# neuromodulation/py_neuromodulation

Hardware: AMD Instinct MI355X
Metric: windows/sec (all features), 256 ch @ 1 kHz (higher is better)
Workload: dtype f32; 1 GPU; 256ch/GPU @1kHz, W=1000, hop=100, 1024 hops/step, all 9 hot-path features, 4 bands, notch50+CAR, z-score normalisation; channels_per_gpu=256, features_per_window=9984, parallelism=channel-shard x1, no collective

## Files before the change

### py_neuromodulation_amd/csrc/nmx_api.hip

```cpp
#include <chrono>
#include <map>
#include <unordered_map>
#include <thread>
#include <hip/hip_runtime.h>

#include "nmx_k_bank.h"
#include "nmx_k_bank_w64.h"
#include "nmx_k_bank_w64d.h"
#include "nmx_k_bank_w64e.h"
#include "nmx_k_bursts.h"
#include "nmx_k_burst_fill.h"
#include "nmx_k_kalman.h"
#include "nmx_k_norm.h"
#include "nmx_k_power.h"
#include "nmx_k_prep.h"
#include "nmx_k_rawnorm.h"
#include "nmx_k_resample.h"
#include "nmx_k_resample64.h"
#include "nmx_k_sharpwave.h"
#include "nmx_k_specmm.h"
#include "nmx_k_timeosc.h"
#include "nmx_k_timeosc_w510.h"

#include <cstdlib>
#include <map>
#include <mutex>
#include <string>

extern __shared__ __attribute__((aligned(16))) float nmx_smem[];

__global__ void __launch_bounds__(256) nmx_kern_timeosc(const NmxTimeOscArgs A) {
  const int item = blockIdx.x;
  nmx_time_osc_item(A, item / A.n_channels, item % A.n_channels, nmx_smem);
}
__global__ void __launch_bounds__(256) nmx_kern_bank(const NmxBankArgs A, int n_items) {
  for (int item = blockIdx.x; item < n_items; item += gridDim.x)
    nmx_bank_item(A, item / A.n_channels, item % A.n_channels, nmx_smem, (int)blockIdx.x);
}
template <int CH>
__global__ void __launch_bounds__(256) nmx_kern_burst_thr(const NmxBurstThrArgs A) {
  __builtin_amdgcn_s_setprio(3);
  const int item = blockIdx.x;
  nmx_burst_thr_item<CH>(A, item / A.n_bands, item % A.n_bands, nmx_smem);
}
__global__ void __launch_bounds__(NMX_FILL_NT) nmx_kern_burst_fill(const NmxBurstThrArgs A, int n2, unsigned short* slots) {
  const int item = blockIdx.x;
  nmx_burst_fill_item(A, item / A.n_bands, item % A.n_bands, n2, slots, nmx_smem);
}
__global__ void __launch_bounds__(NMX_FILL_NT) nmx_kern_burst_fill_sort(const NmxBurstThrArgs A, int n2, unsigned short* slots, float* sorted) {
  const int item = blockIdx.x;
  nmx_burst_fill_sort_item(A, item / A.n_bands, item % A.n_bands, n2, slots, sorted, nmx_smem);
}
__global__ void __launch_bounds__(64) nmx_kern_burst_fill_walk(const NmxBurstThrArgs A, int n2, const unsigned short* slots, const float* sorted) {
  const int item = blockIdx.x;
  nmx_burst_fill_walk_item(A, item / A.n_bands, item % A.n_bands, n2, slots, sorted, nmx_smem);
}
__global__ void __launch_bounds__(1024) nmx_kern_burst_thr_wide(const NmxBurstThrArgs A) {
  const int item = blockIdx.x;
  nmx_burst_thr_item<64>(A, item / A.n_bands, item % A.n_bands, nmx_smem);
}
__global__ void __launch_bounds__(NMX_THR_TILE_NT) nmx_kern_burst_thr_tiled(const NmxBurstThrArgs A) {
  const int item = blockIdx.x;
  nmx_burst_thr_walk<1, true>(A, item / A.n_bands, item % A.n_bands, nmx_smem);
}
extern "C" void nmx_timeosc_fixed_launch128(const NmxTimeOscArgs* A, int n_items, size_t lds, hipStream_t s);
extern "C" void nmx_hilbert_fixed_launch128(const NmxHilbertArgs* A, long long n_items, size_t lds, hipStream_t s);
extern "C" void nmx_wave_launch_burst_stat(const NmxBurstStatArgs* A, NmxBurstStatKind kind, int n_items, size_t lds, hipStream_t s);
extern "C" void nmx_wave_launch_sharp(const NmxSharpArgs* A, int n_items, size_t lds, hipStream_t s);
__global__ void __launch_bounds__(256) nmx_kern_reref(const NmxRerefArgs A) {
  nmx_reref_tile(A, (long long)blockIdx.x * 256 + threadIdx.x, (int)blockIdx.y * NMX_REREF_ROWS);
}
__global__ void __launch_bounds__(256) nmx_kern_resample(const NmxResampleArgs A) {
  const int item = blockIdx.x;
  nmx_resample_item(A, item / A.n_channels, item % A.n_channels, nmx_smem);
}
__global__ void __launch_bounds__(64) nmx_kern_rawnorm_stats(const NmxRawNormArgs A) {
  nmx_rawnorm_stats_item(A, (int)blockIdx.x);
}
__global__ void __launch_bounds__(NMX_RAWNORM_ORDER_NT) nmx_kern_rawnorm_order(const NmxRawNormArgs A) {
  extern __shared__ __attribute__((aligned(16))) float nmx_smem_rn[];
  nmx_rawnorm_order_item(A, (int)blockIdx.x, nmx_smem_rn);
}
__global__ void __launch_bounds__(256) nmx_kern_rawnorm_apply(const NmxRawNormArgs A) {
  nmx_rawnorm_apply(A, (long long)blockIdx.x * 256 + threadIdx.x);
}
__global__ void __launch_bounds__(64) nmx_kern_kalman(const NmxKalmanArgs A) {
  const int i = (int)(blockIdx.x * 64 + threadIdx.x);
  nmx_kalman_item(A, i / A.n_bands, i % A.n_bands);
}
__global__ void __launch_bounds__(64) nmx_kern_norm(const NmxNormArgs A) {
  nmx_norm_column(A, (int)(blockIdx.x * 64 + threadIdx.x));
}
__global__ void __launch_bounds__(64) nmx_kern_norm_seg_hist(const NmxNormArgs A, const NmxNormScan S) {
  nmx_norm_seg_hist(A, S, (int)blockIdx.y, (int)(blockIdx.x * 64 + threadIdx.x));
}
__global__ void __launch_bounds__(64) nmx_kern_norm_seg_batch(const NmxNormArgs A, const NmxNormScan S) {
  nmx_norm_seg_batch(A, S, (int)blockIdx.y, (int)(blockIdx.x * 64 + threadIdx.x));
}
__global__ void __launch_bounds__(64) nmx_kern_norm_seg_offsets(const NmxNormArgs A, const NmxNormScan S) {
  nmx_norm_seg_offsets(A, S, (int)(blockIdx.x * 64 + threadIdx.x));
}
__global__ void __launch_bounds__(256) nmx_kern_norm_cell(const NmxNormArgs A, const NmxNormScan S) {
  nmx_norm_scan_cell(A, S, (int)blockIdx.x, (int)(blockIdx.y * 256 + threadIdx.x));
}
__global__ void __launch_bounds__(256) nmx_kern_norm_ring(const NmxNormArgs A, const NmxNormScan S) {
  nmx_norm_scan_ring(A, S, (int)blockIdx.x, (int)(blockIdx.y * 256 + threadIdx.x));
}
__global__ void __launch_bounds__(256) nmx_kern_power_prep(const NmxPowerPrepArgs P) {
  nmx_power_prep_at(P, (int)blockIdx.x, (int)(blockIdx.y * 256 + threadIdx.x));
}
__global__ void __launch_bounds__(64) nmx_kern_power(const NmxPowerArgs A) {
  nmx_power_cell(A, (int)blockIdx.x, (int)(blockIdx.y * 64 + threadIdx.x));
}
__global__ void __launch_bounds__(256) nmx_kern_power_ring(const NmxPowerPrepArgs P) {
  nmx_power_ring_at(P, (int)blockIdx.x, (int)(blockIdx.y * 256 + threadIdx.x));
}
template <int NW>
__global__ void __launch_bounds__(64 * NW) nmx_kern_car(const NmxCarArgs A) {
  __shared__ double red[64 * NW];
  nmx_car_tile<NW>(A, (long long)blockIdx.x * 64, red);
}
__global__ void __launch_bounds__(256) nmx_kern_reref_struct(const NmxRerefStructArgs A) {
  __shared__ double red[NMX_RS_GROUPS * 256];
  nmx_reref_struct_tile(A, (long long)blockIdx.x * 64, red);
}
__global__ void __launch_bounds__(256) nmx_kern_shift(const NmxShiftArgs A) {
  nmx_shift_sample(A, (long long)blockIdx.x * 256 + threadIdx.x, (int)blockIdx.y);
}
__global__ void __launch_bounds__(64) nmx_kern_nanmask(const NmxNanMaskArgs A) {
  const int item = blockIdx.x;
  nmx_nanmask_item(A, item / A.C_in, item % A.C_in, nmx_smem);
}
__global__ void __launch_bounds__(256) nmx_kern_tap(const NmxTapArgs A) {
  const int item = blockIdx.x;
  nmx_tap_item(A, item / A.C, item % A.C);
}

static thread_local int g_stage = 0;
static thread_local std::string g_stage_kernels[16];
extern "C" void nmxi_note_kernel(const char* name) {
  std::string& s = g_stage_kernels[g_stage & 15];
  if (s.find(name) != std::string::npos) return;
  if (!s.empty()) s += " + ";
  s += name;
}
static void be_stage(int st) { g_stage = st; }
static void be_stage_reset() { for (auto& s : g_stage_kernels) s.clear(); }
static std::string be_stage_kernels(int st) { return g_stage_kernels[st & 15]; }

typedef hipStream_t be_stream_t;
struct be_timer_t {
  hipEvent_t a = nullptr, b = nullptr;
  bool used = false;
};

static thread_local std::string g_be_err;
static thread_local int g_be_rc = 0;
static int nmx_fail(int code, const std::string& msg);
static int be_hip(hipError_t e, const char* what) {
  if (e == hipSuccess) return 0;
  return nmx_fail(NMX_E_HIP, std::string(what) + ": " + hipGetErrorString(e));
}
#define BE_TRY(call) do { hipError_t e_ = (call); if (e_ != hipSuccess && !g_be_rc) g_be_rc = be_hip(e_, #call); } while (0)

static int be_device_count() {
  int n = 0;
  if (hipGetDeviceCount(&n) != hipSuccess) return 0;
  return n;
}
static int be_set_device(int dev) { return be_hip(hipSetDevice(dev), "hipSetDevice"); }
static int be_cu_count(int dev) {
  int n = 0;
  return hipDeviceGetAttribute(&n, hipDeviceAttributeMultiprocessorCount, dev) == hipSuccess && n > 0 ? n : 256;
}
struct NmxDevIdle { void* p; long long gen; };
struct NmxDevPool {
  std::mutex m;
  std::multimap<std::pair<int, size_t>, NmxDevIdle> idle;
  std::map<void*, std::pair<int, size_t>> live;
  size_t cached = 0, cap = 0;
  long long gen = 0;
  bool cap_read = false;
};
static NmxDevPool& be_dev_pool() { static NmxDevPool* p = new NmxDevPool(); return *p; }
static void be_dev_pool_flush(NmxDevPool& D, size_t keep = 0, long long older_than = -1) {
  for (auto it = D.idle.begin(); it != D.idle.end();) {
    const bool old = older_than >= 0 && it->second.gen <= older_than;
    if (!(old || (older_than < 0 && D.cached > keep))) { ++it; continue; }
    (void)hipFree(it->second.p);
    D.cached -= it->first.second;
    it = D.idle.erase(it);
  }
}
static void be_dev_pool_cap(NmxDevPool& D) {
  if (D.cap_read) return;
  const char* v = getenv("NMX_DEVICE_POOL_MB");
  D.cap = (size_t)((v && v[0] >= '0' && v[0] <= '9') ? atoll(v) : 8192) << 20;
  D.cap_read = true;
}
static void* be_alloc(size_t n) {
  NmxDevPool& D = be_dev_pool();
  int dev = 0;
  if (hipGetDevice(&dev) != hipSuccess) dev = 0;
  const size_t want = ((n ? n : 4) + 255) & ~(size_t)255;
  std::lock_guard<std::mutex> lk(D.m);
  be_dev_pool_cap(D);
  auto it = D.idle.find(std::make_pair(dev, want));
  if (it != D.idle.end()) {
    void* p = it->second.p;
    D.idle.erase(it);
    D.cached -= want;
    D.live[p] = std::make_pair(dev, want);
    return p;
  }
  void* p = nullptr;
  if (hipMalloc(&p, want) != hipSuccess) {
    (void)hipGetLastError();
    be_dev_pool_flush(D);
    if (hipMalloc(&p, want) != hipSuccess) { (void)hipGetLastError(); return nullptr; }
  }
  D.live[p] = std::make_pair(dev, want);
  return p;
}
static void be_free(void* p) {
  if (!p) return;
  NmxDevPool& D = be_dev_pool();
  (void)hipDeviceSynchronize();
  std::lock_guard<std::mutex> lk(D.m);
  auto it = D.live.find(p);
  if (it == D.live.end()) { (void)hipFree(p); return; }
  const std::pair<int, size_t> key = it->second;
  D.live.erase(it);
  size_t cap = D.cap;
  if (cap && key.second >= (size_t)(64u << 20)) {
    size_t fr = 0, tot = 0;
    if (hipMemGetInfo(&fr, &tot) == hipSuccess) cap = std::min(cap, (fr + D.cached) / 8);
    else (void)hipGetLastError();
  }
  if (cap && D.cached + key.second <= cap) {
    D.idle.emplace(key, NmxDevIdle{p, D.gen});
    D.cached += key.second;
    return;
  }
  (void)hipFree(p);
}
static void be_dev_pool_age() {
  NmxDevPool& D = be_dev_pool();
  static const long long keep_plans = [] {
    const char* v = getenv("NMX_POOL_KEEP_PLANS");
    return (long long)((v && v[0] >= '0' && v[0] <= '9') ? atoll(v) : 4);
  }();
  std::lock_guard<std::mutex> lk(D.m);
  D.gen += 1;
  if (D.gen > keep_plans) be_dev_pool_flush(D, 0, D.gen - keep_plans - 1);
}
static long long be_dev_pool_trim(long long keep_bytes) {
  NmxDevPool& D = be_dev_pool();
  std::lock_guard<std::mutex> lk(D.m);
  const size_t before = D.cached;
  be_dev_pool_flush(D, keep_bytes > 0 ? (size_t)keep_bytes : 0);
  return (long long)(before - D.cached);
}
static void* be_host_alloc(size_t n) {
  void* p = nullptr;
  if (hipHostMalloc(&p, n, hipHostMallocPortable)    != hipSuccess) return nullptr;
  return p;
}
static void be_host_free(void* p) { (void)hipHostFree(p); }
static void be_h2d_sync(void* d, const void* s, size_t n) { BE_TRY(hipMemcpy(d, s, n, hipMemcpyHostToDevice)); }
static void be_d2h_sync(void* d, const void* s, size_t n) { BE_TRY(hipMemcpy(d, s, n, hipMemcpyDeviceToHost)); }
static void be_memset_sync(void* d, int v, size_t n) { BE_TRY(hipMemset(d, v, n)); }
static void be_h2d_async(void* d, const void* s, size_t n, be_stream_t st) {
  BE_TRY(hipMemcpyAsync(d, s, n, hipMemcpyHostToDevice, st));
}
static void be_d2h_async(void* d, const void* s, size_t n, be_stream_t st) {
  BE_TRY(hipMemcpyAsync(d, s, n, hipMemcpyDeviceToHost, st));
}
static void be_h2d_2d_async(void* d, size_t dpitch, const void* s, size_t spitch, size_t width,
                            size_t height, be_stream_t st) {
  BE_TRY(hipMemcpy2DAsync(d, dpitch, s, spitch, width, height, hipMemcpyHostToDevice, st));
}
static void be_d2h_2d_async(void* d, size_t dpitch, const void* s, size_t spitch, size_t width,
                            size_t height, be_stream_t st) {
  BE_TRY(hipMemcpy2DAsync(d, dpitch, s, spitch, width, height, hipMemcpyDeviceToHost, st));
}
static void be_memset_async(void* d, int v, size_t n, be_stream_t st) { BE_TRY(hipMemsetAsync(d, v, n, st)); }
static void be_host_fn(be_stream_t st, void (*fn)(void*), void* arg) { BE_TRY(hipLaunchHostFunc(st, fn, arg)); }
static int be_sync(be_stream_t st) { return be_hip(hipStreamSynchronize(st), "hipStreamSynchronize"); }
static int be_sync_watch(be_stream_t st, const std::string* kernels, int n_lists) {
  static const double limit = [] {
    const char* v = getenv("NMX_SYNC_TIMEOUT_S");
    return (v && ((v[0] >= '0' && v[0] <= '9') || v[0] == '.')) ? atof(v) : 300.0;
  }();
  const auto t0 = std::chrono::steady_clock::now();
  for (;;) {
    const hipError_t q = hipStreamQuery(st);
    if (q == hipSuccess) return 0;
    if (q != hipErrorNotReady) return be_hip(q, "hipStreamQuery");
    (void)hipGetLastError();
    const double el = std::chrono::duration<double>(std::chrono::steady_clock::now() - t0).count();
    if (limit > 0.0 && el > limit) {
      std::string msg = "the device did not finish a batch within " + std::to_string((int)limit) + " s (NMX_SYNC_TIMEOUT_S); kernels of the last launch sequence:";
      for (int i = 1; i < n_lists; ++i)
        if (kernels && !kernels[i].empty()) msg += " [stage " + std::to_string(i) + ": " + kernels[i] + "]";
      return nmx_fail(NMX_E_HIP, msg);
    }
    if (el > 1e-3) std::this_thread::sleep_for(std::chrono::microseconds(50));
  }
}
static void be_sync_quiet(be_stream_t st) { if (hipStreamSynchronize(st) != hipSuccess) (void)hipGetLastError(); }
struct NmxStreamPool {
  std::mutex mu;
  std::vector<hipStream_t> idle[2];
  std::unordered_map<hipStream_t, int> cls;
};
static NmxStreamPool& be_stream_pool(int dev) {
  static std::mutex mu;
  static std::map<int, NmxStreamPool*> pools;
  std::lock_guard<std::mutex> lk(mu);
  NmxStreamPool*& p = pools[dev];
  if (!p) p = new NmxStreamPool();
  return *p;
}
static int be_stream_pool_cap() {
  static int cap = -1;
  if (cap < 0) { const char* v = getenv("NMX_STREAM_POOL"); cap = v ? std::max(0, atoi(v)) : 32; }
  return cap;
}
static be_stream_t be_stream_make(int klass) {
  int dev = 0;
  (void)hipGetDevice(&dev);
  NmxStreamPool& P = be_stream_pool(dev);
  hipStream_t s = nullptr;
  {
    std::lock_guard<std::mutex> lk(P.mu);
    if (!P.idle[klass].empty()) { s = P.idle[klass].back(); P.idle[klass].pop_back(); P.cls[s] = klass; return s; }
  }
  if (klass == 1) {
    int lo = 0, hi = 0;
    if (!(hipDeviceGetStreamPriorityRange(&lo, &hi) == hipSuccess &&
          hipStreamCreateWithPriority(&s, hipStreamNonBlocking, hi) == hipSuccess)) {
      s = nullptr;
      (void)hipGetLastError();
    }
  }
  if (!s) BE_TRY(hipStreamCreateWithFlags(&s, hipStreamNonBlocking));
  if (s) { std::lock_guard<std::mutex> lk(P.mu); P.cls[s] = klass; }
  return s;
}
static be_stream_t be_stream_create() { return be_stream_make(0); }
static void be_stream_destroy(be_stream_t s) {
  if (!s) return;
  int dev = 0;
  (void)hipGetDevice(&dev);
  NmxStreamPool& P = be_stream_pool(dev);
  {
    std::lock_guard<std::mutex> lk(P.mu);
    auto it = P.cls.find(s);
    if (it != P.cls.end()) {
      const int klass = it->second;
      P.cls.erase(it);
      if ((int)P.idle[klass].size() < be_stream_pool_cap() && hipStreamQuery(s) == hipSuccess) { P.idle[klass].push_back(s); return; }
      (void)hipGetLastError();
    }
  }
  (void)hipStreamDestroy(s);
}
static be_stream_t be_stream_create_high() { return be_stream_make(1); }
typedef hipEvent_t be_event_t;
static void be_event_create(be_event_t& e) { BE_TRY(hipEventCreateWithFlags(&e, hipEventDisableTiming)); }
static void be_event_destroy(be_event_t& e) { if (e) (void)hipEventDestroy(e); }
static void be_event_record(be_event_t& e, be_stream_t s) { BE_TRY(hipEventRecord(e, s)); }
static void be_stream_wait(be_stream_t s, be_event_t& e) { BE_TRY(hipStreamWaitEvent(s, e, 0)); }
static void be_timer_create(be_timer_t& t) {
  BE_TRY(hipEventCreate(&t.a));
  BE_TRY(hipEventCreate(&t.b));
}
static void be_timer_destroy(be_timer_t& t) {
  if (t.a) (void)hipEventDestroy(t.a);
  if (t.b) (void)hipEventDestroy(t.b);
}
static void be_timer_start(be_timer_t& t, be_stream_t s) { BE_TRY(hipEventRecord(t.a, s)); t.used = false; }
static void be_timer_stop(be_timer_t& t, be_stream_t s) { BE_TRY(hipEventRecord(t.b, s)); t.used = true; }
static float be_timer_elapsed(be_timer_t& t) {
  if (!t.used) return 0.f;
  float ms = 0.f;
  if (hipEventSynchronize(t.b) != hipSuccess) return -1.f;
  if (hipEventElapsedTime(&ms, t.a, t.b) != hipSuccess) return -1.f;
  return ms;
}
static int be_check_launch() {
  hipError_t e = hipGetLastError();
  if (e != hipSuccess) return be_hip(e, "kernel launch");
  int rc = g_be_rc;
  g_be_rc = 0;
  return rc;
}

template <typename K>
static void be_allow_lds(K kern) {
  (void)hipFuncSetAttribute((const void*)kern, hipFuncAttributeMaxDynamicSharedMemorySize, 160 * 1024);
}
static void be_init_once() {
  static unsigned long long seen = 0;
  if (!nmx_first_on_device(seen)) return;
  be_allow_lds(nmx_kern_timeosc);
  be_allow_lds(nmx_kern_bank);
  be_allow_lds(nmx_kern_resample);
  be_allow_lds(nmx_kern_burst_thr<32>);
  be_allow_lds(nmx_kern_burst_thr<64>);
  be_allow_lds(nmx_kern_burst_thr<128>);
  be_allow_lds(nmx_kern_burst_thr_wide);
  be_allow_lds(nmx_kern_burst_thr_tiled);
  be_allow_lds(nmx_kern_burst_fill);
  be_allow_lds(nmx_kern_burst_fill_sort);
  be_allow_lds(nmx_kern_rawnorm_order);
}

extern "C" void nmx_wave_launch_scan(const NmxTimeOscArgs* A, int n_items, hipStream_t s);
extern "C" void nmx_wave_launch_timeosc_w1000_low(const NmxTimeOscArgs* A, int n_items, int n_cu, hipStream_t s);
extern "C" void nmx_wave_launch_timeosc_w1000(const NmxTimeOscArgs* A, int n_items, hipStream_t s);
extern "C" void nmx_wave_launch_timeosc_w510(const NmxTimeOscArgs* A, int n_items, hipStream_t s);
extern "C" void nmx_wave_launch_timeosc_stft500(const NmxTimeOscArgs* A, int n_items, hipStream_t s);
extern "C" void nmx_specmm_launch(const NmxTimeOscArgs* A, int n_items, int n_cu, hipStream_t s);
extern "C" void nmx_wave_launch_timeosc_w1000_todo(const NmxTimeOscArgs* A, int n_items, hipStream_t s);
extern "C" void nmx_timeosc_long_launch(const NmxTimeOscArgs* A, int n_items, hipStream_t s);
static void be_launch_timeosc(const NmxTimeOscArgs& A, NmxTimeOscKind kind, int n_items, int nt, size_t lds, int n_cu, be_stream_t s) {
  be_init_once();
  switch (kind) {
    case NMX_TO_SCAN: nmx_wave_launch_scan(&A, n_items, s); return;
    case NMX_TO_SPECMM: nmx_specmm_launch(&A, n_items, n_cu, s); return;
    case NMX_TO_W1000_LOW: nmx_wave_launch_timeosc_w1000_low(&A, n_items, n_cu, s); return;
    case NMX_TO_W1000: nmx_wave_launch_timeosc_w1000(&A, n_items, s); return;
    case NMX_TO_STFT500: nmx_wave_launch_timeosc_stft500(&A, n_items, s); return;
    case NMX_TO_W510: nmx_wave_launch_timeosc_w510(&A, n_items, s); return;
    case NMX_TO_FIXED128: nmx_timeosc_fixed_launch128(&A, n_items, lds, s); return;
    case NMX_TO_LONG: nmx_timeosc_long_launch(&A, n_items, s); return;
    case NMX_TO_GENERIC:
      hipLaunchKernelGGL(nmx_kern_timeosc, dim3(n_items), dim3(nt), lds, s, A);
      nmxi_note_kernel("nmx_kern_timeosc");
      return;
  }
}
static void be_launch_timeosc_redo(const NmxTimeOscArgs& A, int n_items, be_stream_t s) {
  nmx_wave_launch_timeosc_w1000_todo(&A, n_items, s);
}
static void be_launch_bank(const NmxBankArgs& A, int n_items, int nt, size_t lds, be_stream_t s) {
  be_init_once();
  const int grid = (A.partitioned && n_items > NMX_UPS_SLOTS) ? NMX_UPS_SLOTS : n_items;
  hipLaunchKernelGGL(nmx_kern_bank, dim3(grid), dim3(nt), lds, s, A, n_items);
  nmxi_note_kernel("nmx_kern_bank");
}
extern "C" void nmx_w64_launch_rd64(const NmxBankW64Args*, int, size_t, int, hipStream_t);
extern "C" void nmx_w64x2_launch_rd64(const NmxBankW64Args*, int, int, hipStream_t);
extern "C" void nmx_w64c_launch_rd64(const NmxBankW64Args*, int, int, hipStream_t);
extern "C" void nmx_w64d_launch_rd64(const NmxBankW64Args*, int, int, hipStream_t);
extern "C" void nmx_w64e_launch_rd64(const NmxBankW64Args*, int, int, hipStream_t);
extern "C" void nmx_wave_launch_sharp_todo(const NmxSharpArgs* A, int n_items, size_t lds, const unsigned char* todo,
                                           hipStream_t s);
static void be_launch_bank_w64(const NmxBankW64Args& A, int n_items, size_t lds, int n_cu, be_stream_t s) {
  switch ((NmxFirKernel)A.kernel) {
    case NMX_FIR_X2: nmx_w64x2_launch_rd64(&A, n_items, n_cu, s); return;
    case NMX_FIR_PAIR_C: nmx_w64c_launch_rd64(&A, n_items, n_cu, s); return;
    case NMX_FIR_PAIR_D: nmx_w64d_launch_rd64(&A, n_items, n_cu, s); return;
    case NMX_FIR_PAIR_E: nmx_w64e_launch_rd64(&A, n_items, n_cu, s); return;
    case NMX_FIR_ONE: nmx_w64_launch_rd64(&A, n_items, lds, n_cu, s); return;
  }
}
extern "C" void nmx_w64e_launch_fused_rd64(const NmxBankW64Args*, const NmxBankW64Args*, int, int, int, hipStream_t);
static void be_launch_notch_bank_fused(const NmxBankW64Args& F, const NmxBankW64Args& N, bool g_lds, int n_items, int n_cu,
                                       be_stream_t s) {
  nmx_w64e_launch_fused_rd64(&F, &N, g_lds ? 1 : 0, n_items, n_cu, s);
}
extern "C" void nmx_wave_launch_sharp_dense(const NmxSharpArgs* A, NmxSharpKind kind, int n_items, hipStream_t s);
extern "C" void nmx_wave_launch_sharp_slab(const NmxSharpArgs* A, int n_items, const unsigned char* todo, hipStream_t s);
static void be_launch_sharp(const NmxSharpArgs& A, NmxSharpKind kind, int n_items, size_t lds, be_stream_t s) {
  be_init_once();
  switch (kind) {
    case NMX_SHARP_LIST: nmx_wave_launch_sharp(&A, n_items, lds, s); return;
    case NMX_SHARP_SLAB: nmx_wave_launch_sharp_slab(&A, n_items, nullptr, s); return;
    case NMX_SHARP_DENSE_LIST: nmx_wave_launch_sharp_dense(&A, kind, n_items, s); nmx_wave_launch_sharp_todo(&A, n_items, lds, A.todo, s); return;
    case NMX_SHARP_DENSE_SLAB: nmx_wave_launch_sharp_dense(&A, kind, n_items, s); nmx_wave_launch_sharp_slab(&A, n_items, A.todo, s); return;
  }
}
extern "C" void nmx_wave_launch_hilbert_w500(const NmxHilbertArgs* A, long long n_items, hipStream_t s);
extern "C" void nmx_wave_launch_hilbert_w1000(const NmxHilbertArgs* A, long long n_items, hipStream_t s);
extern "C" void nmx_hilbert_long_launch(const NmxHilbertArgs* A, long long n_items, hipStream_t s);
static void be_launch_hilbert(const NmxHilbertArgs& A, NmxHilbertKind kind, long long n_items, size_t lds, be_stream_t s) {
  be_init_once();
  if (kind == NMX_HIL_W500) nmx_wave_launch_hilbert_w500(&A, n_items, s);
  else if (kind == NMX_HIL_W1000) nmx_wave_launch_hilbert_w1000(&A, n_items, s);
  else if (kind == NMX_HIL_LONG) nmx_hilbert_long_launch(&A, n_items, s);
  else nmx_hilbert_fixed_launch128(&A, n_items, lds, s);
}
extern "C" void nmx_wave_launch_burst_thr(const NmxBurstThrArgs* A, int n_items, int nr, bool list_lds, size_t lds, hipStream_t s);
static void be_launch_burst_thr(const NmxBurstThrArgs& A, const NmxBurstWalk& K, const NmxBurstWalkSeg& g, int n_items, int nt, size_t lds,
                                be_stream_t s) {
  be_init_once();
  if (g.kind == NMX_WALK_WAVE) { nmx_wave_launch_burst_thr(&A, n_items, K.nr, g.list_lds, g.list_lds ? K.lds_list : K.lds, s); return; }
  const int chunk = (A.K + nt - 1) / nt;
  if (nmx_burst_thr_tiled(A.K)) { hipLaunchKernelGGL(nmx_kern_burst_thr_tiled, dim3(n_items), dim3(NMX_THR_TILE_NT), lds, s, A); nmxi_note_kernel("nmx_kern_burst_thr_tiled"); }
  else if (nt > 256) { hipLaunchKernelGGL(nmx_kern_burst_thr_wide, dim3(n_items), dim3(1024), lds, s, A); nmxi_note_kernel("nmx_kern_burst_thr_wide"); }
  else if (chunk <= 32) { hipLaunchKernelGGL(nmx_kern_burst_thr<32>, dim3(n_items), dim3(nt), lds, s, A); nmxi_note_kernel("nmx_kern_burst_thr<32>"); }
  else if (chunk <= 64) { hipLaunchKernelGGL(nmx_kern_burst_thr<64>, dim3(n_items), dim3(nt), lds, s, A); nmxi_note_kernel("nmx_kern_burst_thr<64>"); }
  else { hipLaunchKernelGGL(nmx_kern_burst_thr<128>, dim3(n_items), dim3(nt), lds, s, A); nmxi_note_kernel("nmx_kern_burst_thr<128>"); }
}
static void be_launch_burst_fill(const NmxBurstThrArgs& A, int n_items, unsigned short* slots, float* sorted, bool split, be_stream_t s) {
  be_init_once();
  int n2 = 2048;
  while (n2 < A.W + (A.n_windows - 1) * A.overlap) n2 <<= 1;
  const size_t lds_walk = nmx_burst_fill_walk_lds(n2, A.n_windows);
  if (split && lds_walk <= 48 * 1024) {
    hipLaunchKernelGGL(nmx_kern_burst_fill_sort, dim3(n_items), dim3(NMX_FILL_NT), nmx_burst_fill_sort_lds(n2), s, A, n2, slots, sorted);
    hipLaunchKernelGGL(nmx_kern_burst_fill_walk, dim3(n_items), dim3(64), lds_walk, s, A, n2, (const unsigned short*)slots,
                       (const float*)sorted);
    nmxi_note_kernel("nmx_kern_burst_fill_sort");
    nmxi_note_kernel("nmx_kern_burst_fill_walk");
    return;
  }
  hipLaunchKernelGGL(nmx_kern_burst_fill, dim3(n_items), dim3(NMX_FILL_NT), nmx_burst_fill_lds(n2), s, A, n2, slots);
  nmxi_note_kernel("nmx_kern_burst_fill");
}
static void be_launch_burst_stat(const NmxBurstStatArgs& A, NmxBurstStatKind kind, int n_items, size_t lds, be_stream_t s) {
  be_init_once();
  nmx_wave_launch_burst_stat(&A, kind, n_items, lds, s);
}
static void be_launch_reref(const NmxRerefArgs& A, be_stream_t s) {
  dim3 grid((unsigned)((A.T + 255) / 256), (unsigned)((A.C + NMX_REREF_ROWS - 1) / NMX_REREF_ROWS));
  hipLaunchKernelGGL(nmx_kern_reref, grid, dim3(256), 0, s, A);
  nmxi_note_kernel("nmx_kern_reref");
}
static void be_launch_resample(const NmxResampleArgs& A, int n_items, int nt, size_t lds, be_stream_t s) {
  be_init_once();
  hipLaunchKernelGGL(nmx_kern_resample, dim3(n_items), dim3(nt), lds, s, A);
  nmxi_note_kernel("nmx_kern_resample");
}
static void be_launch_rawnorm(const NmxRawNormArgs& A, be_stream_t s) {
  be_init_once();
  if (A.method >= NMX_RAWNORM_MEDIAN && A.method != NMX_RAWNORM_POWER) {
    const size_t lds = A.lists ? (size_t)8 * NMX_RAWNORM_ORDER_NT + 4 * (2 * NMX_RAWNORM_ORDER_NT + 272)
                               : (size_t)24 * A.max_list + 8 * NMX_RAWNORM_ORDER_NT;
    hipLaunchKernelGGL(nmx_kern_rawnorm_order, dim3(A.n_channels), dim3(NMX_RAWNORM_ORDER_NT), lds, s, A);
    const long long n = (long long)A.n_windows * A.n_channels * A.W;
    hipLaunchKernelGGL(nmx_kern_rawnorm_apply, dim3((unsigned)((n + 255) / 256)), dim3(256), 0, s, A);
    nmxi_note_kernel("nmx_kern_rawnorm_order + nmx_kern_rawnorm_apply");
    return;
  }
  hipLaunchKernelGGL(nmx_kern_rawnorm_stats, dim3(A.n_channels), dim3(64), 0, s, A);
  const long long n = (long long)A.n_windows * A.n_channels * A.W;
  hipLaunchKernelGGL(nmx_kern_rawnorm_apply, dim3((unsigned)((n + 255) / 256)), dim3(256), 0, s, A);
  nmxi_note_kernel("nmx_kern_rawnorm_stats + nmx_kern_rawnorm_apply");
}
static void be_launch_kalman(const NmxKalmanArgs& A, be_stream_t s) {
  const int n = A.n_channels * A.n_bands;
  hipLaunchKernelGGL(nmx_kern_kalman, dim3((unsigned)((n + 63) / 64)), dim3(64), 0, s, A);
  nmxi_note_kernel("nmx_kern_kalman");
}
static void be_launch_norm(const NmxNormArgs& A, be_stream_t s) {
  hipLaunchKernelGGL(nmx_kern_norm, dim3((unsigned)((A.n_cols + 63) / 64)), dim3(64), 0, s, A);
}
static void be_launch_norm_scan(const NmxNormArgs& A, const NmxNormScan& S, be_stream_t s) {
  const unsigned cb = (unsigned)((A.n_cols + 63) / 64);
  const dim3 cells((unsigned)A.n_rows, (unsigned)((A.n_cols + 255) / 256));
  if (S.n_hseg) hipLaunchKernelGGL(nmx_kern_norm_seg_hist, dim3(cb, (unsigned)S.n_hseg), dim3(64), 0, s, A, S);
  hipLaunchKernelGGL(nmx_kern_norm_seg_batch, dim3(cb, (unsigned)S.n_bseg), dim3(64), 0, s, A, S);
  hipLaunchKernelGGL(nmx_kern_norm_seg_offsets, dim3(cb), dim3(64), 0, s, A, S);
  hipLaunchKernelGGL(nmx_kern_norm_cell, cells, dim3(256), 0, s, A, S);
  hipLaunchKernelGGL(nmx_kern_norm_ring, cells, dim3(256), 0, s, A, S);
}
static void be_launch_power(const NmxPowerPrepArgs& P, const NmxPowerArgs& A, be_stream_t s) {
  const unsigned gy = (unsigned)((P.n_cols + 255) / 256);
  hipLaunchKernelGGL(nmx_kern_power_prep, dim3((unsigned)(P.have + P.n_rows), gy), dim3(256), 0, s, P);
  hipLaunchKernelGGL(nmx_kern_power, dim3((unsigned)A.n_rows, (unsigned)((A.n_cols + 63) / 64)), dim3(64), 0, s, A);
  hipLaunchKernelGGL(nmx_kern_power_ring, dim3((unsigned)P.n_rows, gy), dim3(256), 0, s, P);
}
static void be_launch_car(const NmxCarArgs& A, be_stream_t s) {
  if (A.T <= 4096 && A.C >= 64) hipLaunchKernelGGL(nmx_kern_car<16>, dim3((unsigned)((A.T + 63) / 64)), dim3(1024), 0, s, A);
  else hipLaunchKernelGGL(nmx_kern_car<4>, dim3((unsigned)((A.T + 63) / 64)), dim3(256), 0, s, A);
  nmxi_note_kernel("nmx_kern_car");
}
static void be_launch_reref_struct(const NmxRerefStructArgs& A, be_stream_t s) {
  hipLaunchKernelGGL(nmx_kern_reref_struct, dim3((unsigned)((A.T + 63) / 64)), dim3(256), 0, s, A);
  nmxi_note_kernel("nmx_kern_reref_struct");
}
static void be_launch_shift(const NmxShiftArgs& A, be_stream_t s) {
  hipLaunchKernelGGL(nmx_kern_shift, dim3((unsigned)((A.T + 255) / 256), (unsigned)A.C), dim3(256), 0, s, A);
  nmxi_note_kernel("nmx_kern_shift");
}
__global__ void __launch_bounds__(256) nmx_kern_reref64(const NmxReref64Args A) {
  nmx_reref64_tile(A, (long long)blockIdx.x * 256 + threadIdx.x, (int)blockIdx.y * NMX_REREF64_ROWS);
}
static void be_launch_reref64(const NmxReref64Args& A, be_stream_t s) {
  hipLaunchKernelGGL(nmx_kern_reref64, dim3((unsigned)((A.T + 255) / 256), (unsigned)((A.C + NMX_REREF64_ROWS - 1) / NMX_REREF64_ROWS)),
                     dim3(256), 0, s, A);
}
__global__ void __launch_bounds__(256) nmx_kern_rs64_elem(const NmxResample64Args A, int mode, const NmxCplx64* src, NmxCplx64* dst) {
  nmx_rs64_elem(A, mode, src, dst, (int)blockIdx.y, (long long)blockIdx.x * 256 + threadIdx.x);
}
__global__ void __launch_bounds__(256) nmx_kern_rs64_pass(const NmxCplx64* src, NmxCplx64* dst, long long ld, long long n, long long ns,
                                                          long long st, int sign) {
  nmx_rs64_pass(src, dst, ld, n, ns, st, sign, (int)blockIdx.y, (long long)blockIdx.x * 256 + threadIdx.x);
}
static void be_launch_rs64_elem(const NmxResample64Args& A, int mode, const NmxCplx64* src, NmxCplx64* dst, long long n, int rows,
                                be_stream_t s) {
  hipLaunchKernelGGL(nmx_kern_rs64_elem, dim3((unsigned)((n + 255) / 256), (unsigned)rows), dim3(256), 0, s, A, mode, src, dst);
}
static void be_launch_rs64_pass(const NmxCplx64* src, NmxCplx64* dst, long long ld, long long n, long long ns, long long st, int sign,
                                int rows, be_stream_t s) {
  hipLaunchKernelGGL(nmx_kern_rs64_pass, dim3((unsigned)((n / 2 + 255) / 256), (unsigned)rows), dim3(256), 0, s, src, dst, ld, n, ns,
                     st, sign);
}
static void be_launch_nanmask(const NmxNanMaskArgs& A, int n_items, be_stream_t s) {
  hipLaunchKernelGGL(nmx_kern_nanmask, dim3(n_items), dim3(64), 64 * sizeof(float), s, A);
}
static void be_launch_tap(const NmxTapArgs& A, int n_items, be_stream_t s) {
  hipLaunchKernelGGL(nmx_kern_tap, dim3(n_items), dim3(256), 0, s, A);
}

#include "nmx_engine.inc"
```

### py_neuromodulation_amd/csrc/nmx_common.h

```cpp
#pragma once

#include <math.h>
#include <stdint.h>

#ifdef NMX_HOST_EMU
struct float2 {
  float x, y;
};
static inline float2 make_float2(float x, float y) { return float2{x, y}; }
#define NMX_DEV static inline
#define NMX_DEVM inline
#define NMX_TID 0
#define NMX_NT 1
#define NMX_SYNC() ((void)0)
#define NMX_GLOBAL_FENCE() ((void)0)
#define NMX_RESTRICT
#else
#include <hip/hip_runtime.h>
#define NMX_DEV __device__ __forceinline__
#define NMX_DEVM __device__ __forceinline__
#ifdef NMX_NT_FIXED
#define NMX_TID ((int)(threadIdx.x & 63))
#define NMX_NT 64
#elif defined(NMX_BLOCK_FIXED)
#define NMX_TID ((int)threadIdx.x)
#define NMX_NT NMX_BLOCK_FIXED
#else
#define NMX_TID ((int)threadIdx.x)
#define NMX_NT ((int)blockDim.x)
#endif
#define NMX_WAVE_FENCE() asm volatile("s_waitcnt lgkmcnt(0)" ::: "memory")
#if defined(NMX_NT_FIXED) && defined(NMX_SYNC_GLOBAL)
#define NMX_SYNC()                                                       \
  do {                                                                   \
    __builtin_amdgcn_fence(__ATOMIC_ACQ_REL, "workgroup");               \
    asm volatile("s_waitcnt vmcnt(0) lgkmcnt(0)" ::: "memory");          \
  } while (0)
#elif defined(NMX_NT_FIXED)
#define NMX_SYNC() NMX_WAVE_FENCE()
#elif defined(NMX_BLOCK_FIXED)
#define NMX_SYNC()                                        \
  do {                                                    \
    if (NMX_BLOCK_FIXED <= 64) { NMX_WAVE_FENCE(); }      \
    else { __syncthreads(); }                             \
  } while (0)
#else
#define NMX_SYNC()                                   \
  do {                                               \
    if (blockDim.x <= 64) { NMX_WAVE_FENCE(); }      \
    else { __syncthreads(); }                        \
  } while (0)
#endif
#define NMX_RESTRICT __restrict__
#define NMX_GLOBAL_FENCE() __threadfence_block()
extern "C" void nmxi_note_kernel(const char* name);
static inline bool nmx_first_on_device(unsigned long long& seen) {
  int d = 0;
  if (hipGetDevice(&d) != hipSuccess || d < 0 || d > 63) return true;
  if ((seen >> d) & 1ull) return false;
  seen |= 1ull << d;
  return true;
}
#endif

#ifdef NMX_HOST_EMU
static inline int nmx_uniform_i(int v) { return v; }
static inline long long nmx_uniform_ll(long long v) { return v; }
#else
__device__ __forceinline__ int nmx_uniform_i(int v) { return __builtin_amdgcn_readfirstlane(v); }
__device__ __forceinline__ long long nmx_uniform_ll(long long v) {
  const unsigned lo = (unsigned)__builtin_amdgcn_readfirstlane((int)(unsigned)(v & 0xffffffffll));
  const unsigned hi = (unsigned)__builtin_amdgcn_readfirstlane((int)(unsigned)((unsigned long long)v >> 32));
  return (long long)(((unsigned long long)hi << 32) | lo);
}
#endif

#define NMX_MAX_STAGES 12
#define NMX_MAX_BANDS_DEV 16
#define NMX_SMM_NG 63
#define NMX_SMM_TAB_FLOATS (4 * NMX_SMM_NG * 64)
#define NMX_MAX_FILTERS_DEV 24
#define NMX_MAX_SW_COMBOS_DEV 48

struct NmxFftStage {
  int radix;
  int ns;
  int m;
  unsigned magic;
  int tw_step;
};

struct NmxFft {
  int n;
  int nstages;
  NmxFftStage st[NMX_MAX_STAGES];
  const float2* tw;
  const float2* twr;
};

struct NmxCols {
  int base, ch_stride, a_stride, b_stride;
};

struct NmxOsc {
  int enabled;
  int n;
  int nfreq;
  int k_lo, k_hi;
  int nseg;
  int step;
  int half;
  int complex_full;
  int log_transform;
  unsigned estimators;
  int n_est;
  int return_spectrum;
  float scale;
  float log10_scale;
  int bin_lo[NMX_MAX_BANDS_DEV], bin_hi[NMX_MAX_BANDS_DEV];
  float inv_bins[NMX_MAX_BANDS_DEV];
  NmxCols cols, psd_cols;
  NmxFft fft;
  const float* win;
  const float2* wdc;
  int nadd;
  int split_d, sub_m;
  const float2* tw_n;
};

struct NmxTimeOscArgs {
  int stft_per_wave;
  const float* x;
  long long ch_stride;
  long long win_stride;
  const long long* starts;
  float* out;
  int n_outputs;
  int n_channels;
  int W;
  int n_bands;
  int clean_on_load;
  unsigned features;
  NmxCols hjorth_cols, raw_cols, ll_cols;
  NmxOsc fft, welch, stft;
  int off_x, off_a, off_b, off_spec, off_red, lds_floats;
  const float* w500_tab;
  const unsigned short* w510_tab;
  const float* smm_tab;
  int smm_k0;
  int starts_mod4;
  const float* dcf;
  unsigned short* todo;
  int long_mode;
  int long_nb;
  int long_spec_slab;
  int slab_floats;
  int slab_blocks;
  float* slab;
};

enum NmxTimeOscKind { NMX_TO_SCAN, NMX_TO_SPECMM, NMX_TO_W1000_LOW, NMX_TO_W1000, NMX_TO_STFT500, NMX_TO_W510, NMX_TO_FIXED128, NMX_TO_GENERIC, NMX_TO_LONG };
enum NmxHilbertKind { NMX_HIL_W500, NMX_HIL_W1000, NMX_HIL_FIXED128, NMX_HIL_LONG };
enum NmxBurstStatKind { NMX_BSTAT_REG16, NMX_BSTAT_REG16_SPARSE, NMX_BSTAT_REG32, NMX_BSTAT_REG32_SPARSE, NMX_BSTAT_GENERIC, NMX_BSTAT_SCAN };
enum NmxSharpKind { NMX_SHARP_LIST, NMX_SHARP_DENSE_LIST, NMX_SHARP_SLAB, NMX_SHARP_DENSE_SLAB };
enum NmxFirKernel { NMX_FIR_ONE, NMX_FIR_X2, NMX_FIR_PAIR_C, NMX_FIR_PAIR_D, NMX_FIR_PAIR_E };

#define NMXD_F_HJORTH (1u << 0)
#define NMXD_F_RAW (1u << 1)
#define NMXD_F_BANDPOWER (1u << 2)
#define NMXD_F_STFT (1u << 3)
#define NMXD_F_FFT (1u << 4)
#define NMXD_F_WELCH (1u << 5)
#define NMXD_F_SHARPWAVE (1u << 6)
#define NMXD_F_BURSTS (1u << 7)
#define NMXD_F_LINELENGTH (1u << 8)

#define NMXD_EST_MEAN 1u
#define NMXD_EST_MEDIAN 2u
#define NMXD_EST_STD 4u
#define NMXD_EST_MAX 8u
```

### py_neuromodulation_amd/csrc/nmx_engine.inc

```

#include <algorithm>
#include <chrono>
#include <cmath>
#include <cstdio>
#include <cstdlib>
#include <cstring>
#include <map>
#include <string>
#include <thread>
#include <deque>
#include <functional>
#include <mutex>
#include <condition_variable>
#include <pthread.h>
#include <vector>

#include "../../include/nmx.h"
#include "nmx_k_coh.h"
#include "nmx_k_proj.h"

static thread_local std::string g_nmx_err;
static int nmx_fail(int code, const std::string& msg) {
  g_nmx_err = msg;
  return code;
}
#define NMX_REQUIRE(cond, msg) \
  do { if (!(cond)) return nmx_fail(NMX_E_INVALID, std::string(msg)); } while (0)

#ifdef NMX_HOST_EMU
static void be_launch_timeosc(const NmxTimeOscArgs& A, NmxTimeOscKind, int n, int nt, size_t lds, int, be_stream_t s) { be_launch_timeosc(A, n, nt, lds, s); }
static void be_launch_hilbert(const NmxHilbertArgs& A, NmxHilbertKind, long long n, size_t lds, be_stream_t s) { be_launch_hilbert(A, n, 128, lds, s); }
static void be_launch_bank_w64(const NmxBankW64Args& A, int n, size_t lds, int, be_stream_t s) { be_launch_bank_w64(A, n, lds, s); }
static void be_launch_burst_thr(const NmxBurstThrArgs& A, const NmxBurstWalk&, const NmxBurstWalkSeg&, int n, int nt, size_t lds, be_stream_t s) {
  be_launch_burst_thr(A, n, nt, lds, s);
}
static void be_launch_burst_fill(const NmxBurstThrArgs& A, int n, unsigned short* slots, float* sorted, bool, be_stream_t s) {
  be_launch_burst_fill(A, n, slots, sorted, s);
}
static void be_launch_burst_stat(const NmxBurstStatArgs& A, NmxBurstStatKind, int n, size_t lds, be_stream_t s) { be_launch_burst_stat(A, n, lds, s); }
static void be_launch_sharp(const NmxSharpArgs& A, NmxSharpKind, int n, size_t lds, be_stream_t s) { be_launch_sharp(A, n, lds, s); }
static int be_cu_count(int) { return 256; }
#endif

namespace {

constexpr double kPi = 3.14159265358979323846;

template <void* (*Alloc)(size_t), void (*Free)(void*)>
struct Block {
  void* p = nullptr;
  size_t cap = 0;
  Block() = default;
  Block(const Block&) = delete;
  Block& operator=(const Block&) = delete;
  ~Block() { if (p) Free(p); }
  bool regrow(size_t bytes) {
    if (p) Free(p);
    p = Alloc(bytes);
    cap = p ? bytes : 0;
    return p != nullptr;
  }
};
using Buf = Block<be_alloc, be_free>;
using HostBuf = Block<be_host_alloc, be_host_free>;

#include "nmx_engine_sched.inc"

enum Stage {
  ST_BATCH = 0,
  ST_PREP = 1,
  ST_TIMEOSC = 2,
  ST_BANK = 3,
  ST_BURSTS = 4,
  ST_SHARP = 5,
  ST_BANK2 = 6,
  ST_COH = 7,
  ST_PROJ = 8,
  ST_COUNT
};

struct WinView {
  const float* x;
  long long ch_stride, win_stride;
  const long long* starts;
  int clean;
};
template <class Args>
void view_into(Args& A, const WinView& v) {
  A.x = v.x; A.ch_stride = v.ch_stride; A.win_stride = v.win_stride; A.starts = v.starts; A.clean_on_load = v.clean;
}
void view_into(NmxTapArgs& A, const WinView& v) {
  A.x = v.x; A.ch_stride = v.ch_stride; A.win_stride = v.win_stride; A.starts = v.starts; A.clean = v.clean;
}
WinView dense_view(const void* y, int C, int w) { return WinView{(const float*)y, w, (long long)C * w, nullptr, 0}; }

struct FrontStage {
  float* d_R = nullptr;
  bool car = false;
  float car_diag = 0.f, car_off = 0.f;
  bool structured = false;
  NmxRerefStructArgs rst{};
  Buf x_ref;
};
struct TimeOscStage {
  NmxTimeOscArgs a{};
  NmxTimeOscKind kind = NMX_TO_GENERIC;
  bool takes_dc = true;
  int nt = 64;
  Buf todo;
};
struct CohStage {
  NmxCohArgs a{};
};
struct ResampleStage {
  NmxResampleArgs a{};
  int nt = 256;
  Buf y;
};

struct FirLaunch {
  unsigned mask = 0;
  Stage stage = ST_BANK;
  NmxFirKernel kernel = NMX_FIR_ONE;
  bool pipelined = false;
  const float* hc = nullptr;
  const float* twc = nullptr;
  bool fused = false;
};
struct FirStage {
  NmxBankArgs a{};
  bool w64 = false;
  NmxBankW64Args w{};
  std::vector<FirLaunch> launches;
  bool takes_dc = true;
};

struct BurstStage {
  NmxHilbertArgs hil{};
  NmxBurstThrArgs bthr{};
  NmxBurstStatArgs bstat{};
  NmxHilbertKind hil_kind = NMX_HIL_FIXED128;
  bool own_hilbert = false;
  bool sparse = false;
  bool sparse_count = false;
  long long env_tail_rows = 0, env_rows = 0;
  NmxBurstStatKind stat_kind = NMX_BSTAT_GENERIC;
  NmxBurstWalk walk{};
  bool fill_split = true;
  int nt_thr = 256;
  long long seen = 0;
  float* d_top = nullptr;
  long long* d_counts = nullptr;
  size_t top_bytes = 0, counts_bytes = 0;
  float* d_floor = nullptr;
  Buf env[2], thr[2];
  Buf env_full[2];
  Buf yb;
  Buf slots;
  int fill_hops(int nw) const { return walk.fill && seen == 0 ? nmx_burst_fill_hops(bthr, nw) : 0; }
};
struct SharpStage {
  NmxSharpArgs a{};
  NmxSharpKind kind = NMX_SHARP_LIST;
  Buf swy[2], todo[2];
  Buf slab;
};
struct KalmanStage {
  NmxKalmanArgs a{};
  double* d_state = nullptr;
  size_t bytes = 0;
};
struct RawNormStage {
  NmxRawNormArgs a{};
  long long hops = 0;
  bool sorted_valid = false;
  size_t ring_bytes = 0, cnt_bytes = 0, len_bytes = 0;
  Buf x_rn, mean, scale;
  Buf qt, qn;
};

struct Plan {
  nmx_plan_desc d;
  std::vector<std::vector<double>> taps;
  std::vector<double> notch_taps, ref_matrix;
  std::vector<double> notch_taps_used;
  int device = 0;
  int n_cu = 256;
  Schedule sched;
  int host_chunk_windows = 512;
  int host_first_chunk = 128;
  int norm_chunk_windows = 384;
  std::vector<void*> tables;
  ~Plan() { for (void* t : tables) be_free(t); }
  std::map<int, NmxFft> fft_cache;
  std::map<int, const float2*> twn_cache;
  FrontStage front;
  FirStage bank;
  bool have_bank = false;
  FirStage notch;
  bool have_notch = false;
  int notch_bank_fuse = 0;
  std::vector<FirStage> pre;
  const float* w64e_tw = nullptr;
  const float* w500_tab = nullptr;
  BurstStage bursts;
  bool have_bursts = false;
  SharpStage sharp;
  bool have_sharp = false;
  TimeOscStage timeosc;
  bool have_timeosc = false;
  CohStage coherence;
  bool have_coh = false;
  int nt_bank = 256;
  int chunk_windows = 1024;
  int burst_handoff_mb = 2048;
  bool tiny_inline = true;
  bool starts_mod4 = false;
  Buf tap;
  Buf x_in, x_in2[2], x_pf[2], y_notch, out, starts, mask;
  HostBuf win_pin;
  KalmanStage kalman;
  bool have_kalman = false;
  ResampleStage resample;
  bool have_resample = false;
  RawNormStage rawnorm;
  bool have_rawnorm = false;
  std::vector<std::vector<double>> pre_taps;
  int w_in = 0;
  be_timer_t timers[ST_COUNT];
  std::string kernels[ST_COUNT];
  nmx_norm* norm = nullptr;
  nmx_proj* proj = nullptr;
  bool dc_ok = false;
  bool dc_auto = true;
  bool dc_host_set = false, dc_learned = false, dc_dirty = false;
  bool dc_active = false;
  bool dc_sub_active = false;
  double dc_gain = 1.0;
  std::vector<double> dc_host;
  std::vector<float> dc_sub_h;
  std::vector<double> dc_pre_h;
  float* d_dc_sub = nullptr;
  float* d_dc_pref = nullptr;
  float* d_dc_nanv = nullptr;
  Buf x_dc;
  const volatile int64_t* pipe_in_ready = nullptr;
  volatile int64_t* pipe_out_done = nullptr;
  struct Progress { volatile int64_t* dst; int64_t value; };
  std::vector<Progress> pipe_marks;
};

static thread_local double g_ensure_scale = 1.0;
int ensure(Buf& b, size_t bytes) {
  if (bytes <= b.cap) return 0;
  if (g_ensure_scale > 1.0) bytes = (size_t)((double)bytes * g_ensure_scale) + 256;
  const size_t want = bytes + bytes / 8;
  if (!b.regrow(want)) return nmx_fail(NMX_E_NOMEM, "device allocation of " + std::to_string(want) + " bytes failed");
  return 0;
}

void* plan_alloc(Plan& P, size_t bytes) {
  void* d = be_alloc(bytes ? bytes : 4);
  if (d) P.tables.push_back(d);
  return d;
}
void* upload(Plan& P, const void* src, size_t bytes) {
  void* d = plan_alloc(P, bytes);
  if (d && bytes) be_h2d_sync(d, src, bytes);
  return d;
}

int env_int(const char* name, int dflt) {
  const char* v = getenv(name);
  return (v && v[0] >= '0' && v[0] <= '9') ? atoi(v) : dflt;
}

#include "nmx_engine_dc.inc"
#include "nmx_engine_plan_spectral.inc"
#include "nmx_engine_plan_bursts.inc"
#include "nmx_engine_plan_fir.inc"
#include "nmx_engine_plan_state.inc"

}

#include "nmx_engine_abi.inc"
#include "nmx_engine_run.inc"
#include "nmx_engine_norm.inc"
#include "nmx_engine_proj.inc"
#include "nmx_engine_host.inc"
```

### py_neuromodulation_amd/csrc/nmx_engine_run.inc

```
static int run_prep_stages(Plan& P, WinView& v, int nw, be_stream_t s, const NmxBankArgs* fuse_bank = nullptr) {
  const int C = P.d.n_channels, Wi = P.w_in;
  int rc;
  for (size_t i = 0; i < P.pre.size(); ++i) {
    Buf& dst = P.x_pf[i & 1];
    if ((rc = ensure(dst, (size_t)nw * C * Wi * sizeof(float)))) return rc;
    NmxBankArgs A = P.pre[i].a;
    view_into(A, v);
    A.out = nullptr; A.sw_out = (float*)dst.p;
    launch_fir_stage(P, P.pre[i], A, nw * C, s);
    v = dense_view(dst.p, C, Wi);
  }
  if (P.have_notch) {
    if ((rc = ensure(P.y_notch, (size_t)nw * C * Wi * sizeof(float)))) return rc;
    NmxBankArgs A = P.notch.a;
    view_into(A, v);
    A.out = nullptr; A.y_out = (float*)P.y_notch.p;
#ifndef NMX_HOST_EMU
    if (fuse_bank) launch_notch_bank_fused(P, A, *fuse_bank, nw * C, s);
    else
#endif
    launch_fir_stage(P, P.notch, A, nw * C, s);
    v = dense_view(P.y_notch.p, C, Wi);
  }
  if (P.have_resample && (rc = launch_resample(P, v, nw, s))) return rc;
  if (P.have_rawnorm && (rc = run_rawnorm(P, v, nw, s))) return rc;
  return 0;
}

static int run_chunk(Plan& P, const BatchSched& b, const float* d_x, long long ldx, long long lo, long long hi,
                     const long long* d_starts, int nw, float* d_out, bool timed, float* d_pre = nullptr,
                     const int64_t* h_starts = nullptr, be_event_t* samples_free = nullptr, bool* samples_freed = nullptr) {
  const nmx_plan_desc& d = P.d;
  const int C = d.n_channels, W = d.window;
  const be_stream_t s = b.s;
  int rc;
  const int par = P.sched.parity();
  P.sched.begin_chunk(b);
  Buf& B_env = P.bursts.env[par];
  Buf& B_swy = P.sharp.swy[par];
  WinView v{d_x, ldx, 0, d_starts, 1};
  const bool tev = timed && nw >= 8;
  if (timed) be_stage_reset();
  if (tev) be_timer_start(P.timers[ST_PREP], s);
  be_stage(ST_PREP);
  if ((rc = launch_front(P, d_x, ldx, lo, hi - lo, true, s, v))) return rc;
  bool raw_live = v.x == d_x;
  if (h_starts) {
    long long hop = nw > 1 ? (long long)(h_starts[1] - h_starts[0]) : 0;
    for (int i = 2; i < nw && hop >= 0; ++i)
      if ((long long)(h_starts[i] - h_starts[i - 1]) != hop) hop = -1;
    if (hop >= 0) { v.x += h_starts[0]; v.win_stride = hop; v.starts = nullptr; }
  }
  NmxBankArgs fuse_a{};
  if (P.notch_bank_fuse) {
    fuse_a = P.bank.a;
    fuse_a.out = d_out;
    fuse_a.dcf = dc_table(P);
    if (P.have_sharp) {
      if ((rc = ensure(B_swy, (size_t)nw * C * d.n_sw_filters * W * sizeof(float)))) return rc;
      fuse_a.sw_out = (float*)B_swy.p;
    }
  }
  if ((rc = run_prep_stages(P, v, nw, s, P.notch_bank_fuse ? &fuse_a : nullptr))) return rc;
  if (!P.pre.empty() || P.have_notch || P.have_resample || P.have_rawnorm) raw_live = false;
  if (d_pre) {
    NmxTapArgs T{};
    view_into(T, v);
    T.y = d_pre; T.C = C; T.W = W;
    be_launch_tap(T, nw * C, s);
  }
  if (tev) be_timer_stop(P.timers[ST_PREP], s);
  const bool freed = !raw_live && samples_free;
  if (freed) be_event_record(*samples_free, s);
  if (samples_freed) *samples_freed = freed;
  bool dc_made = false;
  be_stage(ST_BANK);
  if (P.have_bank) {
    NmxBankArgs A = P.bank.a;
    A.out = d_out;
    if ((rc = dc_bind(P, A, P.bank.takes_dc, v, nw, s, dc_made))) return rc;
    if (P.have_bursts) {
      if ((rc = ensure(B_env, (size_t)nw * C * d.n_burst_bands * W * sizeof(float)))) return rc;
      A.env_out = (float*)B_env.p;
    }
    if (P.have_sharp) {
      if ((rc = ensure(B_swy, (size_t)nw * C * d.n_sw_filters * W * sizeof(float)))) return rc;
      A.sw_out = (float*)B_swy.p;
    }
    if (P.have_bursts && P.bursts.own_hilbert) {
      if ((rc = ensure(P.bursts.yb, (size_t)nw * C * d.n_burst_bands * W * sizeof(float)))) return rc;
      A.yb_out = (float*)P.bursts.yb.p;
    }
    launch_fir_stage(P, P.bank, A, nw * C, s, tev);
    launch_kalman(P, nw, d_out, s);
  }
  const bool sharp_side = P.sched.sharp_on_side(b);
  if (sharp_side) {
    if ((rc = launch_sharp_stage(P, par, nw, d_out, P.sched.fork_sharp(b), tev))) return rc;
    P.sched.join_sharp();
  }
  be_stage(ST_BURSTS);
  if (P.have_bursts && (rc = launch_burst_stage(P, b, nw, d_out, tev))) return rc;
  if ((rc = launch_timeosc_stage(P, v, nw, d_out, s, tev, dc_made))) return rc;
  launch_coh_stage(P, v, nw, d_out, s, tev);
  if (!sharp_side && (rc = launch_sharp_stage(P, par, nw, d_out, s, tev))) return rc;
  P.sched.end_main(b);
  be_stage(ST_BATCH);
  if (timed) for (int i = 0; i < ST_PROJ; ++i) P.kernels[i] = be_stage_kernels(i);
  return be_check_launch();
}

static int proj_launch(nmx_proj* proj, float* rows, long long ld, int n_rows, be_stream_t s);
static bool plan_finalizes(const Plan& P) { return P.norm || P.proj; }
static int chunk_finalize(Plan& P, const BatchSched& b, float* d_outk, int ld, int nw, bool timed) {
  int rc = 0;
  if (timed) P.kernels[ST_PROJ].clear();
  if (plan_finalizes(P)) {
    be_stream_t sf = P.sched.begin_finalize(b);
    if (P.norm) rc = nmx_norm_process(P.norm, d_outk, ld, nw, 1, (void*)sf);
    if (P.proj && !rc) {
      const bool tev = timed && nw >= 8;
      if (tev) be_timer_start(P.timers[ST_PROJ], sf);
      if (timed) { be_stage_reset(); be_stage(ST_PROJ); }
      rc = proj_launch(P.proj, d_outk, ld, nw, sf);
      if (tev) be_timer_stop(P.timers[ST_PROJ], sf);
      if (timed) { P.kernels[ST_PROJ] = be_stage_kernels(ST_PROJ); be_stage(ST_BATCH); }
    }
    P.sched.end_finalize(sf);
  }
  P.sched.next_chunk();
  return rc;
}

static int check_batch_args(Plan* P, const float* x, int64_t ldx, int64_t n_samples, const int64_t* starts, int64_t n_windows,
                            float* out, int memspace) {
  if (!P || !x || !starts || !out) return nmx_fail(NMX_E_INVALID, "null argument");
  NMX_REQUIRE(n_windows >= 1, "n_windows must be >= 1");
  NMX_REQUIRE(memspace == 0 || memspace == 1, "memspace must be 0 (host) or 1 (device)");
  NMX_REQUIRE(ldx >= n_samples && n_samples >= P->w_in, "ldx / n_samples too small");
  bool mod4 = true;
  for (int64_t i = 0; i < n_windows; ++i) {
    NMX_REQUIRE(starts[i] >= 0 && starts[i] + P->w_in <= n_samples, "window outside the data");
    mod4 = mod4 && (starts[i] & 3) == 0;
  }
  P->starts_mod4 = mod4;
  return 0;
}

struct ChunkSizes {
  bool host;
  int64_t dev_chunk, host_first, host_big;
  int64_t at(int64_t w0) const { return host ? (w0 == 0 ? host_first : host_big) : dev_chunk; }
};
static ChunkSizes batch_chunk_sizes(const Plan& P, bool host) {
  ChunkSizes z{host, 0, 0, 0};
  const bool no_handoff = !P.have_bank && !P.have_notch && !P.front.d_R && !P.have_resample && !P.have_rawnorm && P.pre.empty();
  z.dev_chunk = no_handoff ? (int64_t)P.chunk_windows * 16
                           : (P.norm ? std::min<int64_t>(P.chunk_windows, P.norm_chunk_windows) : (int64_t)P.chunk_windows);
  z.host_big = std::min<int64_t>(P.chunk_windows, P.host_chunk_windows);
  z.host_first = std::min<int64_t>(z.host_big, P.host_first_chunk);
  if (host && P.have_bursts)
    z.host_first = std::max<int64_t>(z.host_first, P.bursts.fill_hops((int)z.host_big));
  if (P.have_bursts && P.d.window > 16384) {
    const double per_hop = 3.0 * P.d.n_channels * P.d.n_burst_bands * (double)P.d.window * sizeof(float);
    const int64_t cap = std::max<int64_t>(1, (int64_t)((double)P.burst_handoff_mb * 1048576.0 / per_hop));
    z.dev_chunk = std::min(z.dev_chunk, cap);
    z.host_big = std::min(z.host_big, cap);
    z.host_first = std::min(z.host_first, cap);
  }
  return z;
}

static int stage_host_chunk(Plan& P, const BatchSched& b, int k, const float* x, int64_t ldx, long long lo, long long hi,
                            const float** d_xk, long long* ldxk) {
  const int Cin = P.d.n_channels_in;
  const be_stream_t sc = P.sched.in_stream(b);
  Buf& xb = P.x_in2[k & 1];
  const long long n_range = hi - lo;
  int rc;
  if ((rc = ensure(xb, (size_t)Cin * n_range * sizeof(float)))) return rc;
  P.sched.wait_input_free(b, k, plan_finalizes(P));
  if (P.pipe_in_ready) {
    long long pos = lo, spins = 0;
    while (pos < hi) {
      const long long want = std::min<long long>(hi, pos + 4096);
      long long ready = __atomic_load_n(P.pipe_in_ready, __ATOMIC_ACQUIRE);
      if (ready < want) {
        if (++spins > 2000000) return nmx_fail(NMX_E_INVALID, "nmx_plan_set_pipeline: the input never became ready");
        std::this_thread::sleep_for(std::chrono::microseconds(5));
        continue;
      }
      const long long upto = std::min<long long>(hi, ready);
      be_h2d_2d_async((float*)xb.p + (pos - lo), (size_t)n_range * sizeof(float), x + pos, (size_t)ldx * sizeof(float),
                      (size_t)(upto - pos) * sizeof(float), (size_t)Cin, sc);
      pos = upto;
    }
  } else {
    be_h2d_2d_async(xb.p, (size_t)n_range * sizeof(float), x + lo, (size_t)ldx * sizeof(float),
                    (size_t)n_range * sizeof(float), (size_t)Cin, sc);
  }
  P.sched.input_copied(b);
  *d_xk = (const float*)xb.p - lo;
  *ldxk = n_range;
  return 0;
}

struct BatchOut {
  float *out, *d_out;
  uint8_t* nan_mask;
  unsigned char* d_mask;
  int F, Cin;
};
static void fetch_back(Plan& P, const BatchSched& b, const BatchOut& o, int64_t w0, int64_t nw, int par) {
  const be_stream_t so = P.sched.out_stream(b);
  if (!b.inline_all) P.sched.wait_done(b, so, par, plan_finalizes(P), false);
  be_d2h_async(o.out + (size_t)w0 * o.F, o.d_out + (size_t)w0 * o.F, (size_t)nw * o.F * sizeof(float), so);
  if (o.nan_mask) be_d2h_async(o.nan_mask + (size_t)w0 * o.Cin, o.d_mask + (size_t)w0 * o.Cin, (size_t)nw * o.Cin, so);
  if (P.pipe_out_done && P.pipe_marks.size() < P.pipe_marks.capacity()) {
    P.pipe_marks.push_back(Plan::Progress{P.pipe_out_done, w0 + nw});
    be_host_fn(so, [](void* a) { auto* m = (Plan::Progress*)a; __atomic_store_n(m->dst, m->value, __ATOMIC_RELEASE); },
               &P.pipe_marks.back());
  }
}

static int process_batch_impl(nmx_plan* plan, const float* x, int64_t ldx, int64_t n_samples,
                              const int64_t* starts, int64_t n_windows, float* out, uint8_t* nan_mask,
                              int memspace, void* hip_stream, float* pre) {
  int rc = check_batch_args((Plan*)plan, x, ldx, n_samples, starts, n_windows, out, memspace);
  if (rc) return rc;
  Plan& P = *(Plan*)plan;
  const nmx_plan_desc& d = P.d;
  if ((rc = be_set_device(P.device))) return rc;
  const bool host = memspace == 0;
  const bool tiny = P.tiny_inline && host && n_windows < 8 && !P.pipe_in_ready && !P.pipe_out_done;
  const BatchSched b{hip_stream ? (be_stream_t)hip_stream : P.sched.main, tiny};
  const be_stream_t s = b.s;
  P.sched.last_stream = s;
  BatchOut o{out, out, nan_mask, nan_mask, d.n_outputs + d.n_extra_cols, d.n_channels_in};
  if ((rc = dc_prepare(P, x, ldx, starts[0], host, s))) return rc;
  if ((rc = ensure(P.starts, (size_t)n_windows * sizeof(long long)))) return rc;
  be_h2d_async(P.starts.p, starts, (size_t)n_windows * sizeof(long long), s);
  if (host) {
    if ((rc = ensure(P.out, (size_t)n_windows * o.F * sizeof(float)))) return rc;
    o.d_out = (float*)P.out.p;
    if (nan_mask) {
      if ((rc = ensure(P.mask, (size_t)n_windows * o.Cin))) return rc;
      o.d_mask = (unsigned char*)P.mask.p;
    }
  }
  const ChunkSizes sizes = batch_chunk_sizes(P, host);
  be_timer_start(P.timers[ST_BATCH], s);
  int64_t prev_w0 = -1, prev_nw = 0;
  int k = 0, last_par = -1;
  P.pipe_marks.clear();
  P.pipe_marks.reserve((size_t)(n_windows / std::max<int64_t>(1, std::min<int64_t>({P.host_first_chunk, P.chunk_windows, sizes.dev_chunk,
                                                                                    sizes.host_first, sizes.host_big})) + 8));
  auto bail = [&](int r) {
    P.sched.drain(b);
    return r;
  };
  struct ScaleGuard { ~ScaleGuard() { g_ensure_scale = 1.0; } } scale_guard;
  for (int64_t w0 = 0; w0 < n_windows; ++k) {
    const int nw = (int)std::min<int64_t>(sizes.at(w0), n_windows - w0);
    g_ensure_scale = (host && w0 == 0 && n_windows > nw) ? (double)std::min<int64_t>(sizes.host_big, n_windows - nw) / (double)nw : 1.0;
    long long lo = starts[w0], hi = starts[w0] + P.w_in;
    for (int64_t i = w0; i < w0 + nw; ++i) {
      lo = std::min<long long>(lo, starts[i]);
      hi = std::max<long long>(hi, starts[i] + P.w_in);
    }
    const float* d_xk = x;
    long long ldxk = ldx;
    if (host && (rc = stage_host_chunk(P, b, k, x, ldx, lo, hi, &d_xk, &ldxk))) return bail(rc);
    float* d_outk = o.d_out + (size_t)w0 * o.F;
    be_memset_async(d_outk, 0xFF, (size_t)nw * o.F * sizeof(float), s);
    if (o.d_mask) {
      NmxNanMaskArgs M{};
      M.x = d_xk; M.ldx = ldxk; M.starts = (const long long*)P.starts.p + w0; M.mask = o.d_mask + (size_t)w0 * o.Cin;
      M.C_in = o.Cin; M.W = P.w_in;
      be_launch_nanmask(M, nw * o.Cin, s);
    }
    float* d_prek = nullptr;
    const size_t pre_n = (size_t)nw * d.n_channels * d.window;
    if (pre) {
      if (host) {
        if ((rc = ensure(P.tap, pre_n * sizeof(float)))) return bail(rc);
        d_prek = (float*)P.tap.p;
      } else {
        d_prek = pre + (size_t)w0 * d.n_channels * d.window;
      }
    }
    bool freed = false;
    rc = run_chunk(P, b, d_xk, ldxk, lo, hi, (const long long*)P.starts.p + w0, nw, d_outk, w0 == 0, d_prek, starts + w0,
                   host ? P.sched.input_consumed_event(b, k) : nullptr, &freed);
    if (rc) return bail(rc);
    if (host) P.sched.input_consumed(k, freed);
    if (pre && host)
      be_d2h_async(pre + (size_t)w0 * d.n_channels * d.window, d_prek, pre_n * sizeof(float), s);
    const int par_k = P.sched.parity();
    if ((rc = chunk_finalize(P, b, d_outk, o.F, nw, w0 == 0))) return bail(rc);
    last_par = par_k;
    if (host) {
      if (prev_w0 >= 0) fetch_back(P, b, o, prev_w0, prev_nw, par_k ^ 1);
      prev_w0 = w0;
      prev_nw = nw;
    }
    w0 += nw;
  }
  if (last_par >= 0 && !tiny) P.sched.wait_done(b, s, last_par, plan_finalizes(P), true);
  be_timer_stop(P.timers[ST_BATCH], s);
  if (host) {
    fetch_back(P, b, o, prev_w0, prev_nw, last_par);
    for (be_stream_t st : {P.sched.out_stream(b), P.sched.in_stream(b), s})
      if ((rc = be_sync_watch(st, P.kernels, ST_COUNT))) return rc;
    if (P.pipe_out_done) __atomic_store_n(P.pipe_out_done, (int64_t)n_windows, __ATOMIC_RELEASE);
  }
  return be_check_launch();
}

int nmx_process_batch(nmx_plan* plan, const float* x, int64_t ldx, int64_t n_samples,
                      const int64_t* starts, int64_t n_windows, float* out, uint8_t* nan_mask,
                      int memspace, void* hip_stream) {
  return process_batch_impl(plan, x, ldx, n_samples, starts, n_windows, out, nan_mask, memspace, hip_stream, nullptr);
}

int nmx_process_batch_tap(nmx_plan* plan, const float* x, int64_t ldx, int64_t n_samples,
                          const int64_t* starts, int64_t n_windows, float* out, uint8_t* nan_mask,
                          int memspace, void* hip_stream, float* pre) {
  if (!pre) return nmx_fail(NMX_E_INVALID, "null argument");
  return process_batch_impl(plan, x, ldx, n_samples, starts, n_windows, out, nan_mask, memspace, hip_stream, pre);
}

int nmx_process_window(nmx_plan* plan, const double* x, int64_t ldx, float* out, uint8_t* nan_mask) {
  Plan* P = (Plan*)plan;
  if (!P || !x || !out) return nmx_fail(NMX_E_INVALID, "null argument");
  const int Cin = P->d.n_channels_in, W = P->w_in, F = P->d.n_outputs + P->d.n_extra_cols;
  const size_t xb = (((size_t)Cin * W * sizeof(float)) + 255) & ~(size_t)255, ob = (((size_t)F * sizeof(float)) + 255) & ~(size_t)255;
  const size_t need = xb + ob + (size_t)Cin;
  if (P->win_pin.cap < need) {
    int rc = be_set_device(P->device);
    if (rc) return rc;
    if (!P->win_pin.regrow(need)) return nmx_fail(NMX_E_NOMEM, "page-locked host allocation failed");
  }
  float* xf = (float*)P->win_pin.p;
  float* of = (float*)((char*)P->win_pin.p + xb);
  uint8_t* mf = (uint8_t*)P->win_pin.p + xb + ob;
  for (int c = 0; c < Cin; ++c) {
    const double dh = P->dc_host_set ? P->dc_host[c] : 0.0;
    const double* xr = x + (size_t)c * ldx;
    float* d = xf + (size_t)c * W;
    for (int i = 0; i < W; ++i) d[i] = (float)(xr[i] - dh);
  }
  const int64_t start = 0;
  const int rc = nmx_process_batch(plan, xf, W, W, &start, 1, of, nan_mask ? mf : nullptr, 0, nullptr);
  if (rc) return rc;
  memcpy(out, of, (size_t)F * sizeof(float));
  if (nan_mask) memcpy(nan_mask, mf, (size_t)Cin);
  return 0;
}

int nmx_preprocess_window(nmx_plan* plan, const double* x, int64_t ldx, double* y, int64_t ldy) {
  Plan* Pp = (Plan*)plan;
  if (!Pp || !x || !y) return nmx_fail(NMX_E_INVALID, "null argument");
  Plan& P = *Pp;
  const nmx_plan_desc& d = P.d;
  const int Cin = d.n_channels_in, C = d.n_channels, Wo = d.window;
  const int W = P.w_in;
  int rc = be_set_device(P.device);
  if (rc) return rc;
  be_stream_t s = P.sched.main;
  std::vector<float> xf((size_t)Cin * W), yf((size_t)C * Wo);
  for (int c = 0; c < Cin; ++c) {
    const double dh = P.dc_host_set ? P.dc_host[c] : 0.0;
    for (int i = 0; i < W; ++i) {
      const double v = x[(size_t)c * ldx + i];
      xf[(size_t)c * W + i] = (float)((v != v ? 0.0 : v) - dh);
    }
  }
  if ((rc = dc_prepare(P, xf.data(), W, 0, true, s))) return rc;
  if ((rc = ensure(P.x_in, xf.size() * sizeof(float)))) return rc;
  be_h2d_async(P.x_in.p, xf.data(), xf.size() * sizeof(float), s);
  NMX_REQUIRE(P.front.d_R || Cin == C, "n_channels_in != n_channels without ref_matrix");
  WinView v{(const float*)P.x_in.p, W, 0, nullptr, 1};
  be_stage_reset();
  be_stage(ST_PREP);
  if ((rc = launch_front(P, v.x, W, 0, W, false, s, v))) return rc;
  if ((rc = run_prep_stages(P, v, 1, s))) return rc;
  be_stage(ST_BATCH);
  for (int i = 0; i < ST_PROJ; ++i) P.kernels[i] = be_stage_kernels(i);
  be_d2h_async(yf.data(), v.x, yf.size() * sizeof(float), s);
  if ((rc = be_sync(s))) return rc;
  for (int c = 0; c < C; ++c)
    for (int i = 0; i < Wo; ++i) {
      float f = yf[(size_t)c * Wo + i];
      if (v.clean) f = (f != f) ? 0.f : f;
      y[(size_t)c * ldy + i] = (double)f + (P.dc_active ? P.dc_pre_h[c] : 0.0);
    }
  return be_check_launch();
}

int nmx_filter_window(nmx_plan* plan, const double* x, int64_t ldx, double* y) {
  Plan* Pp = (Plan*)plan;
  if (!Pp || !x || !y) return nmx_fail(NMX_E_INVALID, "null argument");
  Plan& P = *Pp;
  NMX_REQUIRE(P.have_bank, "plan has no FIR bank");
  const nmx_plan_desc& d = P.d;
  const int C = d.n_channels, W = d.window, NF = d.n_filters;
  int rc = be_set_device(P.device);
  if (rc) return rc;
  be_stream_t s = P.sched.main;
  std::vector<float> xf((size_t)C * W), yf((size_t)C * NF * W);
  for (int c = 0; c < C; ++c)
    for (int i = 0; i < W; ++i) xf[(size_t)c * W + i] = (float)x[(size_t)c * ldx + i];
  if ((rc = ensure(P.x_in, xf.size() * sizeof(float)))) return rc;
  if ((rc = ensure(P.sharp.swy[0], yf.size() * sizeof(float)))) return rc;
  be_h2d_async(P.x_in.p, xf.data(), xf.size() * sizeof(float), s);
  NmxBankArgs A = P.bank.a;
  view_into(A, WinView{(const float*)P.x_in.p, W, 0, nullptr, 0});
  A.out = nullptr;
  A.n_sw_filters = NF; A.sw_out = (float*)P.sharp.swy[0].p;
  for (int i = 0; i < NF; ++i) {
    A.f[i].sw_index = i; A.f[i].bp_seglen = 0; A.f[i].burst_index = -1; A.f[i].store_raw = 0;
  }
  be_stage_reset();
  be_stage(P.bank.launches[0].stage);
  launch_fir_stage(P, P.bank, A, C, s, false, true);
  be_stage(ST_BATCH);
  for (int i = 0; i < ST_PROJ; ++i) P.kernels[i] = be_stage_kernels(i);
  be_d2h_async(yf.data(), P.sharp.swy[0].p, yf.size() * sizeof(float), s);
  if ((rc = be_sync(s))) return rc;
  for (size_t i = 0; i < yf.size(); ++i) y[i] = (double)yf[i];
  return be_check_launch();
}

int nmx_last_timing_ms(nmx_plan* plan, int which, float* ms) {
  Plan* P = (Plan*)plan;
  if (!P || !ms || which < ST_BATCH || which >= ST_COUNT) return nmx_fail(NMX_E_INVALID, "bad argument");
  be_set_device(P->device);
  *ms = be_timer_elapsed(P->timers[which]);
  return 0;
}


int nmx_host_alloc(int64_t n_bytes, void** out) {
  if (!out || n_bytes < 0) return nmx_fail(NMX_E_INVALID, "bad argument");
  if (be_device_count() <= 0) return nmx_fail(NMX_E_NODEVICE, "no HIP device");
  *out = be_host_alloc((size_t)n_bytes);
  if (!*out) return nmx_fail(NMX_E_NOMEM, "page-locked host allocation of " + std::to_string(n_bytes) + " bytes failed");
  return 0;
}
int nmx_host_free(void* p) {
  if (p) be_host_free(p);
  return 0;
}
int nmx_device_pool_trim(int64_t keep_bytes, int64_t* freed) {
  if (keep_bytes < 0) return nmx_fail(NMX_E_INVALID, "keep_bytes must be >= 0");
  const long long n = be_dev_pool_trim((long long)keep_bytes);
  if (freed) *freed = (int64_t)n;
  return 0;
}

int nmx_reref_f64(int device, const double* ref_matrix, int n_out, int n_in, const double* x, int64_t ldx,
                  int64_t n_samples, double* y, int64_t ldy) {
  if (!ref_matrix || !x || !y) return nmx_fail(NMX_E_INVALID, "null argument");
  NMX_REQUIRE(n_out >= 1 && n_in >= 1 && n_samples >= 0 && ldx >= n_samples && ldy >= n_samples,
              "nmx_reref_f64: n_out, n_in >= 1, n_samples >= 0, ldx / ldy >= n_samples");
  if (n_samples == 0) return 0;
  if (be_device_count() <= 0) return nmx_fail(NMX_E_NODEVICE, "no HIP device");
  int rc = be_set_device(device);
  if (rc) return rc;
  const size_t T = (size_t)n_samples, nR = (size_t)n_out * n_in * sizeof(double);
  const size_t nx = (size_t)n_in * T * sizeof(double), ny = (size_t)n_out * T * sizeof(double);
  char* d = (char*)be_alloc(nR + nx + ny);
  if (!d) return nmx_fail(NMX_E_NOMEM, "nmx_reref_f64: device allocation of " + std::to_string(nR + nx + ny) + " bytes failed");
  be_stream_t s = be_stream_create();
  be_h2d_async(d, ref_matrix, nR, s);
  be_h2d_2d_async(d + nR, T * sizeof(double), x, (size_t)ldx * sizeof(double), T * sizeof(double), (size_t)n_in, s);
  NmxReref64Args A{};
  A.R = (const double*)d; A.x = (const double*)(d + nR); A.ldx = (long long)T; A.y = (double*)(d + nR + nx); A.ldy = (long long)T;
  A.C = n_out; A.C_in = n_in; A.T = (long long)T;
  be_launch_reref64(A, s);
  be_d2h_2d_async(y, (size_t)ldy * sizeof(double), d + nR + nx, T * sizeof(double), T * sizeof(double), (size_t)n_out, s);
  rc = be_sync(s);
  be_stream_destroy(s);
  be_free(d);
  return rc ? rc : be_check_launch();
}

int nmx_resample_f64(int device, const double* x, int64_t ldx, int n_channels, int64_t n_samples, double ratio, double* y,
                     int64_t ldy, int64_t n_out) {
  if (!x || !y) return nmx_fail(NMX_E_INVALID, "null argument");
  NMX_REQUIRE(n_channels >= 1 && n_samples >= 1 && n_samples <= (1ll << 24) && ldx >= n_samples,
              "nmx_resample_f64: n_channels >= 1, 1 <= n_samples <= 2^24, ldx >= n_samples");
  NMX_REQUIRE(ratio > 0 && ratio != 1.0 && ratio <= 1024.0, "nmx_resample_f64: ratio must be in (0, 1024] and != 1");
  const long long W = n_samples, final_len = (long long)std::nearbyint(ratio * (double)W);
  NMX_REQUIRE(final_len == n_out && ldy >= n_out, "nmx_resample_f64: n_out must equal round(ratio * n_samples) and ldy >= n_out");
  if (final_len == 0) return 0;
  const long long min_add = std::min<long long>(W / 8, 100) * 2;
  long long n_pad = 1;
  while (n_pad < W + min_add) n_pad <<= 1;
  const long long pad_l = (n_pad - W) / 2;
  const long long n_new = std::max<long long>((long long)std::nearbyint(ratio * (double)n_pad), 1);
  const long long crop_l = (long long)std::nearbyint(ratio * (double)pad_l);
  NMX_REQUIRE(crop_l + final_len <= n_new, "internal: resample crop outside the output");
  NMX_REQUIRE(n_new <= (1ll << 28), "nmx_resample_f64: resampled padded length beyond 2^28 samples");
  long long L = 0;
  if (n_new & (n_new - 1)) { L = 1; while (L < 2 * n_new - 1) L <<= 1; }
  if (be_device_count() <= 0) return nmx_fail(NMX_E_NODEVICE, "no HIP device");
  int rc = be_set_device(device);
  if (rc) return rc;
  const int C = n_channels;
  const long long ld = std::max(std::max(n_pad, n_new), L);
  const size_t nx = (size_t)C * W * sizeof(double), ny = (size_t)C * final_len * sizeof(double);
  const size_t nw = (size_t)C * ld * sizeof(NmxCplx64), nc = (size_t)L * sizeof(NmxCplx64);
  char* d = (char*)be_alloc(nx + ny + 2 * nw + 2 * nc);
  if (!d) return nmx_fail(NMX_E_NOMEM, "nmx_resample_f64: device allocation of " + std::to_string(nx + ny + 2 * nw + 2 * nc) + " bytes failed");
  be_stream_t s = be_stream_create();
  NmxResample64Args A{};
  A.x = (const double*)d; A.ldx = W; A.y = (double*)(d + nx); A.ldy = final_len;
  A.a = (NmxCplx64*)(d + nx + ny); A.b = (NmxCplx64*)(d + nx + ny + nw); A.ld = ld; A.C = C;
  A.W = W; A.W_new = final_len; A.n_pad = n_pad; A.pad_l = pad_l; A.n_new = n_new; A.crop_l = crop_l; A.L = L;
  const long long use_len = std::min(n_new, n_pad);
  A.nyq_bin = (use_len % 2 == 0) ? use_len / 2 : -1;
  A.nyq_scale = n_new < n_pad ? 2.0 : 0.5;
  A.scale = ratio / (double)n_new / (L ? (double)L : 1.0);
  be_h2d_2d_async(d, (size_t)W * sizeof(double), x, (size_t)ldx * sizeof(double), (size_t)W * sizeof(double), (size_t)C, s);
  auto fft = [&](NmxCplx64*& cur, NmxCplx64*& oth, long long ldr, long long n, int sign, int rows) {
    for (long long ns = n, st = 1; ns > 1; ns >>= 1, st <<= 1) {
      be_launch_rs64_pass(cur, oth, ldr, n, ns, st, sign, rows, s);
      std::swap(cur, oth);
    }
  };
  NmxCplx64 *cur = A.a, *oth = A.b;
  be_launch_rs64_elem(A, NMX_RS64_PAD, nullptr, cur, n_pad, C, s);
  fft(cur, oth, ld, n_pad, -1, C);
  be_launch_rs64_elem(A, NMX_RS64_MAP, cur, oth, L ? L : n_new, C, s);
  std::swap(cur, oth);
  if (!L) {
    fft(cur, oth, ld, n_new, +1, C);
  } else {
    NmxCplx64 *cc = (NmxCplx64*)(d + nx + ny + 2 * nw), *co = cc + L;
    be_launch_rs64_elem(A, NMX_RS64_CHIRP, nullptr, cc, L, 1, s);
    fft(cc, co, L, L, -1, 1);
    A.chirp = cc;
    fft(cur, oth, ld, L, -1, C);
    be_launch_rs64_elem(A, NMX_RS64_MUL, nullptr, cur, L, C, s);
    fft(cur, oth, ld, L, +1, C);
  }
  be_launch_rs64_elem(A, NMX_RS64_OUT, cur, nullptr, final_len, C, s);
  be_d2h_2d_async(y, (size_t)ldy * sizeof(double), d + nx, (size_t)final_len * sizeof(double), (size_t)final_len * sizeof(double),
                  (size_t)C, s);
  rc = be_sync(s);
  be_stream_destroy(s);
  be_free(d);
  return rc ? rc : be_check_launch();
}

int nmx_last_kernels(nmx_plan* plan, int which, char* buf, int64_t n) {
  Plan* P = (Plan*)plan;
  if (!P || !buf || n < 1 || which < ST_PREP || which >= ST_COUNT) return nmx_fail(NMX_E_INVALID, "bad argument");
  std::string k = P->kernels[which];
  if (which == ST_BURSTS && P->bursts.sparse_count)
    k += (k.empty() ? "" : ",") + std::string("env_tail_rows=") + std::to_string(P->bursts.env_tail_rows) + "/" + std::to_string(P->bursts.env_rows);
  const size_t m = std::min<size_t>(k.size(), (size_t)n - 1);
  memcpy(buf, k.data(), m);
  buf[m] = 0;
  return 0;
}
```

### py_neuromodulation_amd/csrc/nmx_k_bank_w64c.h

```cpp
#pragma once

#include "nmx_k_bank_w64.h"

#define NMX_W64C_M 1536
#define NMX_W64C_TILE_FLOATS (2 * 24 * 72)
#define NMX_W64C_TWA_FLOATS (2 * 24 * 64)
#define NMX_W64C_TWB_FLOATS (2 * 8 * 8)
#define NMX_W64C_H_FLOATS 1536

static inline bool nmx_w64_pair_shape_ok(const NmxBankArgs& b) { return b.W <= 1024 && !(b.bp_features & 6u); }
static inline int nmx_w64_pair_waves(int fixed, int tile) { return (NMX_W64_LDS_FLOATS - fixed) / tile; }
static inline int nmx_w64c_fixed(int n_filters) { return n_filters * NMX_W64C_H_FLOATS + NMX_W64C_TWA_FLOATS; }
static inline bool nmx_w64c_fits(int n_filters) {
  return n_filters >= 1 && nmx_w64_pair_waves(nmx_w64c_fixed(n_filters), NMX_W64C_TILE_FLOATS) >= 6;
}

#if !defined(NMX_HOST_EMU) && defined(NMX_LDS_ASM)

template <int OFF>
NMX_DEV void nmx_ds_write_b64(unsigned addr, nmx_c2 v) {
  *(__attribute__((address_space(3))) volatile nmx_c2*)((__attribute__((address_space(3))) volatile char*)(unsigned long)addr + OFF) = v;
}
NMX_DEV nmx_c2 nmx_pk_mul_k(nmx_c2 a, float k) {
  const nmx_c2 kk = {k, k};
  nmx_c2 r;
  asm("v_pk_mul_f32 %0, %1, %2" : "=v"(r) : "v"(a), "s"(kk));
  return r;
}
template <int CONJ>
NMX_DEV nmx_c2 nmx_cmul_k(nmx_c2 a, float wr, float wi) {
  const nmx_c2 w = {wr, wi};
  nmx_c2 t, r;
  asm("v_pk_mul_f32 %0, %1, %2 op_sel_hi:[1,0]" : "=v"(t) : "v"(a), "s"(w));
  if (CONJ)
    asm("v_pk_fma_f32 %0, %1, %2, %3 op_sel:[1,1,0] op_sel_hi:[0,1,1] neg_hi:[0,1,0]" : "=v"(r) : "v"(a), "s"(w), "v"(t));
  else
    asm("v_pk_fma_f32 %0, %1, %2, %3 op_sel:[1,1,0] op_sel_hi:[0,1,1] neg_lo:[0,1,0]" : "=v"(r) : "v"(a), "s"(w), "v"(t));
  return r;
}
NMX_DEV nmx_c2 nmx_pk_mul_lo(nmx_c2 z, nmx_c2 h) {
  nmx_c2 r;
  asm("v_pk_mul_f32 %0, %1, %2 op_sel_hi:[1,0]" : "=v"(r) : "v"(z), "v"(h));
  return r;
}
NMX_DEV nmx_c2 nmx_pk_mul_hi(nmx_c2 z, nmx_c2 h) {
  nmx_c2 r;
  asm("v_pk_mul_f32 %0, %1, %2 op_sel:[0,1] op_sel_hi:[1,1]" : "=v"(r) : "v"(z), "v"(h));
  return r;
}

#define NMX_K_H8 0.70710678118654752f
#define NMX_K_S3 0.86602540378443865f

template <int DIR, int MM>
NMX_DEV nmx_c2 nmx_mul_w24(nmx_c2 a) {
  constexpr float C[15] = {1.f, 0.96592582628906829f, 0.86602540378443865f, 0.70710678118654752f, 0.5f,
                           0.25881904510252076f, 0.f, -0.25881904510252076f, -0.5f, -0.70710678118654752f,
                           -0.86602540378443865f, -0.96592582628906829f, -1.f, -0.96592582628906829f, -0.86602540378443865f};
  constexpr float S[15] = {0.f, 0.25881904510252076f, 0.5f, 0.70710678118654752f, 0.86602540378443865f,
                           0.96592582628906829f, 1.f, 0.96592582628906829f, 0.86602540378443865f, 0.70710678118654752f,
                           0.5f, 0.25881904510252076f, 0.f, -0.25881904510252076f, -0.5f};
  if constexpr (MM == 0) return a;
  else if constexpr (MM == 6) return nmx_mul_i<DIR>(a);
  else if constexpr (MM == 12) return -a;
  else if constexpr (MM == 3) return nmx_pk_mul_k(nmx_add_ib<DIR>(a, a), NMX_K_H8);
  else return nmx_cmul_k<(DIR < 0)>(a, C[MM], S[MM]);
}

template <int DIR>
NMX_DEV void nmx_dft8(nmx_c2* a) {
  const nmx_c2 s0 = a[0] + a[4], d0 = a[0] - a[4];
  const nmx_c2 s1 = a[1] + a[5], d1 = a[1] - a[5];
  const nmx_c2 s2 = a[2] + a[6], d2 = a[2] - a[6];
  const nmx_c2 s3 = a[3] + a[7], d3 = a[3] - a[7];
  {
    const nmx_c2 t0 = s0 + s2, t1 = s0 - s2, t2 = s1 + s3, t3 = s1 - s3;
    a[0] = t0 + t2;
    a[4] = t0 - t2;
    a[2] = nmx_add_ib<DIR>(t1, t3);
    a[6] = nmx_add_ib<-DIR>(t1, t3);
  }
  {
    const nmx_c2 e1 = nmx_pk_mul_k(nmx_add_ib<DIR>(d1, d1), NMX_K_H8);
    const nmx_c2 f3 = nmx_pk_mul_k(nmx_add_ib<-DIR>(d3, d3), NMX_K_H8);
    const nmx_c2 t0 = nmx_add_ib<DIR>(d0, d2), t1 = nmx_add_ib<-DIR>(d0, d2);
    const nmx_c2 t2 = e1 - f3, t3 = e1 + f3;
    a[1] = t0 + t2;
    a[5] = t0 - t2;
    a[3] = nmx_add_ib<DIR>(t1, t3);
    a[7] = nmx_add_ib<-DIR>(t1, t3);
  }
}

template <int JA>
NMX_DEV void nmx_dft24_fwd_col(nmx_c2* v) {
  const nmx_c2 a0 = v[JA], a1 = v[JA + 8];
  const nmx_c2 d = nmx_pk_mul_k(a1, NMX_K_S3);
  const nmx_c2 m = nmx_c2_fma(a1, nmx_mk2(-0.5f, -0.5f), a0);
  v[JA] = a0 + a1;
  v[JA + 8] = nmx_mul_w24<-1, JA>(nmx_add_ib<-1>(m, d));
  v[JA + 16] = nmx_mul_w24<-1, 2 * JA>(nmx_add_ib<+1>(m, d));
}
NMX_DEV void nmx_dft24_fwd(nmx_c2* v) {
  nmx_dft24_fwd_col<0>(v); nmx_dft24_fwd_col<1>(v); nmx_dft24_fwd_col<2>(v); nmx_dft24_fwd_col<3>(v);
  nmx_dft24_fwd_col<4>(v); nmx_dft24_fwd_col<5>(v); nmx_dft24_fwd_col<6>(v); nmx_dft24_fwd_col<7>(v);
  nmx_dft8<-1>(v);
  nmx_dft8<-1>(v + 8);
  nmx_dft8<-1>(v + 16);
}
template <int JA>
NMX_DEV void nmx_dft24_inv_col(nmx_c2* v) {
  const nmx_c2 a0 = v[JA], a1 = nmx_mul_w24<+1, JA>(v[JA + 8]), a2 = nmx_mul_w24<+1, 2 * JA>(v[JA + 16]);
  const nmx_c2 t = a1 + a2, d = nmx_pk_mul_k(a1 - a2, NMX_K_S3);
  const nmx_c2 m = nmx_c2_fma(t, nmx_mk2(-0.5f, -0.5f), a0);
  v[JA] = a0 + t;
  v[JA + 8] = nmx_add_ib<+1>(m, d);
}
NMX_DEV void nmx_dft24_inv(nmx_c2* v) {
  nmx_dft8<+1>(v);
  nmx_dft8<+1>(v + 8);
  nmx_dft8<+1>(v + 16);
  nmx_dft24_inv_col<0>(v); nmx_dft24_inv_col<1>(v); nmx_dft24_inv_col<2>(v); nmx_dft24_inv_col<3>(v);
  nmx_dft24_inv_col<4>(v); nmx_dft24_inv_col<5>(v); nmx_dft24_inv_col<6>(v); nmx_dft24_inv_col<7>(v);
}

constexpr int nmx_w64c_p1(int i) { return 8 * 72 * (3 * (i & 7) + (i >> 3)); }
constexpr int nmx_w64c_p2(int i) { return 8 * (576 * (i >> 3) + 8 * (i & 7)); }
constexpr int nmx_w64c_p3(int i) { return 8 * (576 * (i >> 3) + 9 * (i & 7)); }
constexpr int nmx_w64c_p4(int i) { return 8 * (576 * (i >> 3) + (i & 7)); }
template <int... I> NMX_DEV void nmx_w64c_rd1(nmx_c2* v, unsigned a, std::integer_sequence<int, I...>) { ((v[I] = nmx_ds_read_b64<nmx_w64c_p1(I)>(a)), ...); }
template <int... I> NMX_DEV void nmx_w64c_rd2(nmx_c2* v, unsigned a, std::integer_sequence<int, I...>) { ((v[I] = nmx_ds_read_b64<nmx_w64c_p2(I)>(a)), ...); }
template <int... I> NMX_DEV void nmx_w64c_rd3(nmx_c2* v, unsigned a, std::integer_sequence<int, I...>) { ((v[I] = nmx_ds_read_b64<nmx_w64c_p3(I)>(a)), ...); }
template <int... I> NMX_DEV void nmx_w64c_rd4(nmx_c2* v, unsigned a, std::integer_sequence<int, I...>) { ((v[I] = nmx_ds_read_b64<nmx_w64c_p4(I)>(a)), ...); }
template <int... I> NMX_DEV void nmx_w64c_wr1(const nmx_c2* v, unsigned a, std::integer_sequence<int, I...>) { (nmx_ds_write_b64<nmx_w64c_p1(I)>(a, v[I]), ...); }
template <int... I> NMX_DEV void nmx_w64c_wr2(const nmx_c2* v, unsigned a, std::integer_sequence<int, I...>) { (nmx_ds_write_b64<nmx_w64c_p2(I)>(a, v[I]), ...); }
template <int... I> NMX_DEV void nmx_w64c_wr3(const nmx_c2* v, unsigned a, std::integer_sequence<int, I...>) { (nmx_ds_write_b64<nmx_w64c_p3(I)>(a, v[I]), ...); }
template <int... I> NMX_DEV void nmx_w64c_wr4(const nmx_c2* v, unsigned a, std::integer_sequence<int, I...>) { (nmx_ds_write_b64<nmx_w64c_p4(I)>(a, v[I]), ...); }
template <int... I> NMX_DEV void nmx_w64c_rdt(nmx_c2* v, unsigned a, std::integer_sequence<int, I...>) { ((v[I] = nmx_ds_read_b64<512 * I>(a)), ...); }

struct NmxW64cLane {
  unsigned a1, a2, a4;
  unsigned twa;
  nmx_c2 twb[8];
};
#define NMX_W64C_SEQ24 std::make_integer_sequence<int, 24>{}

NMX_DEV void nmx_w64c_forward(nmx_c2* v, const NmxW64cLane& Ln) {
  nmx_c2 w[24];
  nmx_w64c_rdt(w, Ln.twa, NMX_W64C_SEQ24);
  NMX_SCHED_FENCE();
  nmx_dft24_fwd(v);
  NMX_UNROLL
  for (int i = 1; i < 24; ++i) v[i] = nmx_cmul_tw<0>(v[i], w[i]);
  nmx_w64c_wr1(v, Ln.a1, NMX_W64C_SEQ24);
  NMX_SCHED_FENCE();
  nmx_w64c_rd2(v, Ln.a2, NMX_W64C_SEQ24);
  NMX_SCHED_FENCE();
  NMX_UNROLL
  for (int g = 0; g < 3; ++g) {
    nmx_dft8<-1>(v + 8 * g);
    NMX_UNROLL
    for (int q = 1; q < 8; ++q) v[8 * g + q] = nmx_cmul_tw<0>(v[8 * g + q], Ln.twb[q]);
  }
  nmx_w64c_wr3(v, Ln.a2, NMX_W64C_SEQ24);
  NMX_SCHED_FENCE();
  nmx_w64c_rd4(v, Ln.a4, NMX_W64C_SEQ24);
  NMX_SCHED_FENCE();
  NMX_UNROLL
  for (int g = 0; g < 3; ++g) nmx_dft8<-1>(v + 8 * g);
}
NMX_DEV void nmx_w64c_inverse(nmx_c2* v, const NmxW64cLane& Ln) {
  NMX_UNROLL
  for (int g = 0; g < 3; ++g) {
    nmx_dft8<+1>(v + 8 * g);
    NMX_UNROLL
    for (int q = 1; q < 8; ++q) v[8 * g + q] = nmx_cmul_tw<1>(v[8 * g + q], Ln.twb[q]);
  }
  nmx_w64c_wr4(v, Ln.a4, NMX_W64C_SEQ24);
  NMX_SCHED_FENCE();
  nmx_w64c_rd3(v, Ln.a2, NMX_W64C_SEQ24);
  NMX_SCHED_FENCE();
  NMX_UNROLL
  for (int g = 0; g < 3; ++g) nmx_dft8<+1>(v + 8 * g);
  nmx_w64c_wr2(v, Ln.a2, NMX_W64C_SEQ24);
  NMX_SCHED_FENCE();
  nmx_c2 w[24];
  nmx_w64c_rd1(v, Ln.a1, NMX_W64C_SEQ24);
  nmx_w64c_rdt(w, Ln.twa, NMX_W64C_SEQ24);
  NMX_SCHED_FENCE();
  NMX_UNROLL
  for (int i = 1; i < 24; ++i) v[i] = nmx_cmul_tw<1>(v[i], w[i]);
  nmx_dft24_inv(v);
}

NMX_DEV void nmx_w64c_lane_setup(NmxW64cLane& Ln, const float* tile, const float* twa_lds, const float* twb_glob, int l) {
  const unsigned base = nmx_lds_addr(tile);
  Ln.a1 = base + 8u * (unsigned)l;
  Ln.a2 = base + 8u * (unsigned)((l >> 3) * 72 + (l & 7));
  Ln.a4 = base + 8u * (unsigned)((l >> 3) * 72 + 9 * (l & 7));
  Ln.twa = nmx_lds_addr(twa_lds) + 8u * (unsigned)l;
  const nmx_c2* tb = (const nmx_c2*)twb_glob + (l & 7);
  NMX_UNROLL
  for (int q = 0; q < 8; ++q) Ln.twb[q] = tb[8 * q];
}

NMX_DEV void nmx_w64c_epilogue(const NmxBankW64Args& AA, const NmxFilterDev& F, const nmx_c2* v, int w, int c, int l, bool two,
                               float* out_row) {
  const NmxBankArgs& A = AA.b;
  const int W = A.W;
  if (F.bp_seglen > 0) {
    const unsigned span = (unsigned)F.bp_seglen;
    const int s_l = l - (W - F.bp_seglen);
    nmx_c2 acc = nmx_mk2(0.f, 0.f), acc2 = nmx_mk2(0.f, 0.f);
    NMX_UNROLL
    for (int j = 0; j < 16; ++j) {
      const float mk = (unsigned)(s_l + 64 * j) < span ? 1.f : 0.f;
      const nmx_c2 val = v[j] * mk;
      acc = acc + val;
      acc2 = nmx_c2_fma(val, val, acc2);
    }
    const float inv_n = 1.f / (float)F.bp_seglen;
    float t1 = nmx_wave_reduce(acc.x, 0.f, [](float a_, float b_) { return a_ + b_; });
    float t2 = nmx_wave_reduce(acc.y, 0.f, [](float a_, float b_) { return a_ + b_; });
    const float q1 = nmx_wave_reduce(acc2.x, 0.f, [](float a_, float b_) { return a_ + b_; });
    const float q2 = nmx_wave_reduce(acc2.y, 0.f, [](float a_, float b_) { return a_ + b_; });
    const float mean1 = t1 * inv_n, mean2 = t2 * inv_n;
    t1 = q1 - mean1 * t1;
    t2 = q2 - mean2 * t2;
    if (mean1 * mean1 * (float)F.bp_seglen > 4.f * t1 || mean2 * mean2 * (float)F.bp_seglen > 4.f * t2) {
      nmx_c2 a2 = nmx_mk2(0.f, 0.f);
      const nmx_c2 mm = nmx_mk2(mean1, mean2);
      NMX_UNROLL
      for (int j = 0; j < 16; ++j) {
        const float mk = (unsigned)(s_l + 64 * j) < span ? 1.f : 0.f;
        const nmx_c2 d = (v[j] - mm) * mk;
        a2 = nmx_c2_fma(d, d, a2);
      }
      t1 = nmx_wave_reduce(a2.x, 0.f, [](float a_, float b_) { return a_ + b_; });
      t2 = nmx_wave_reduce(a2.y, 0.f, [](float a_, float b_) { return a_ + b_; });
    }
    if (l < 2 && (l == 0 || two)) {
      const float act = (l == 0 ? t1 : t2) * inv_n;
      const int col = A.bp_cols.base + (c + l) * A.bp_cols.ch_stride + F.bp_band * A.bp_cols.a_stride;
      out_row[col] = nmx_bp_activity(A.bp_log ? log10f(act) : act, (A.bp_kalman_mask >> F.bp_band) & 1u);
    }
  }
  float* dsw = F.sw_index >= 0 ? A.sw_out + (((long long)w * A.n_channels + c) * A.n_sw_filters + F.sw_index) * W : nullptr;
  float* dyb = F.burst_index >= 0 ? AA.yb_out + (((long long)w * A.n_channels + c) * A.n_burst_bands + F.burst_index) * W : nullptr;
  for (int dst = 0; dst < 2; ++dst) {
    float* d = dst ? dyb : dsw;
    if (!d) continue;
    const long long next = (long long)(dst ? A.n_burst_bands : A.n_sw_filters) * W;
    const nmx_rsrc s1 = nmx_make_rsrc(d, 4 * W);
    const nmx_rsrc s2 = nmx_make_rsrc(d + next, two ? 4 * W : 0);
    NMX_UNROLL
    for (int j = 0; j < 16; ++j) {
      __builtin_amdgcn_raw_buffer_store_b32(__float_as_uint(v[j].x), s1, 4 * l + 256 * j, 0, NMX_SERIES_STORE_AUX);
      __builtin_amdgcn_raw_buffer_store_b32(__float_as_uint(v[j].y), s2, 4 * l + 256 * j, 0, NMX_SERIES_STORE_AUX);
    }
  }
}

NMX_DEV void nmx_bank_w64c_item(const NmxBankW64Args& AA, int w, int c, const NmxW64cLane& Ln, const float* htab) {
  w = nmx_uniform_i(w);
  c = nmx_uniform_i(c);
  const NmxBankArgs& A = AA.b;
  const int W = A.W;
  const int l = (int)(threadIdx.x & 63);
  const bool two = c + 1 < A.n_channels;
  float* out_row = A.out ? A.out + (long long)w * A.n_outputs : nullptr;
  const float* src = A.x + (long long)c * A.ch_stride + (long long)w * A.win_stride +
                     (A.starts ? nmx_uniform_ll(A.starts[w]) : 0ll);
  nmx_c2 v[24], z[24];
  NMX_PROF_DECL

  const nmx_rsrc r1 = nmx_make_rsrc(src, 4 * W);
  const nmx_rsrc r2 = nmx_make_rsrc(src + A.ch_stride, two ? 4 * W : 0);
  NMX_UNROLL
  for (int j = 0; j < 16; ++j) {
    v[j].x = __uint_as_float(__builtin_amdgcn_raw_buffer_load_b32(r1, 4 * l + 256 * j, 0, 0));
    v[j].y = __uint_as_float(__builtin_amdgcn_raw_buffer_load_b32(r2, 4 * l + 256 * j, 0, 0));
  }
  if (A.clean_on_load) {
    NMX_UNROLL
    for (int j = 0; j < 16; ++j) v[j] = nmx_mk2(nmx_clean_bl(v[j].x), nmx_clean_bl(v[j].y));
  }
  if (A.dcf) {
    const nmx_c2 dd = nmx_mk2(A.dcf[c], two ? A.dcf[c + 1] : 0.f);
    NMX_UNROLL
    for (int j = 0; j < 16; ++j) {
      if (64 * j + 63 < W) v[j] += dd;
      else if (l + 64 * j < W) v[j] += dd;
    }
  }
  float m1 = 0.f, m2 = 0.f;
  NMX_UNROLL
  for (int j = 0; j < 16; ++j) { m1 = fmaxf(m1, fabsf(v[j].x)); m2 = fmaxf(m2, fabsf(v[j].y)); }
  m1 = nmx_wave_reduce(m1, 0.f, [](float a_, float b_) { return fmaxf(a_, b_); });
  m2 = nmx_wave_reduce(m2, 0.f, [](float a_, float b_) { return fmaxf(a_, b_); });
  int e = 0;
  if (m1 > 0.f && m2 > 0.f) {
    e = __builtin_amdgcn_frexp_expf(m1) - __builtin_amdgcn_frexp_expf(m2);
    e = e < -60 ? -60 : (e > 60 ? 60 : e);
  }
  NMX_UNROLL
  for (int j = 0; j < 16; ++j) v[j].y = __builtin_amdgcn_ldexpf(v[j].y, e);
  const nmx_c2 unscale = nmx_mk2(m1 > 0.f ? 1.f : 0.f, m2 > 0.f ? __builtin_amdgcn_ldexpf(1.f, -e) : 0.f);

  NMX_PROF(0)
  nmx_w64c_forward(v, Ln);
  NMX_UNROLL
  for (int i = 0; i < 24; ++i) z[i] = v[i];
  NMX_PROF(1)

  const int nf = A.n_filters;
  const unsigned h_addr = nmx_lds_addr(htab) + 8u * (unsigned)l;
  for (int fi = 0; fi < nf; ++fi) {
    const NmxFilterDev& F = A.f[fi];
    {
      nmx_c2 h[12];
      nmx_w64c_rdt(h, h_addr + (unsigned)fi * (NMX_W64C_H_FLOATS * 4u), std::make_integer_sequence<int, 12>{});
      NMX_SCHED_FENCE();
      NMX_UNROLL
      for (int i = 0; i < 12; ++i) {
        v[2 * i] = nmx_pk_mul_lo(z[2 * i], h[i]);
        v[2 * i + 1] = nmx_pk_mul_hi(z[2 * i + 1], h[i]);
      }
    }
    NMX_PROF(2)
    nmx_w64c_inverse(v, Ln);
    NMX_UNROLL
    for (int j = 0; j < 16; ++j) v[j] = v[j] * unscale;
    NMX_PROF(3)

    nmx_w64c_epilogue(AA, F, v, w, c, l, two, out_row);
    NMX_PROF(5)
  }
#if defined(NMX_BANK_PROFILE)
  if (w == 5 && (c == 2 || c == 40) && l == 0)
    printf("bank c profile w=%d c=%d: load+scale %lld | forward %lld | spectral %lld | inverse %lld | variance %lld | stores %lld "
           "(cycles, whole item, %d filters)\n", w, c, pf_acc[0], pf_acc[1], pf_acc[2], pf_acc[3], pf_acc[4], pf_acc[5], nf);
#endif
}
#endif
```

### py_neuromodulation_amd/csrc/nmx_k_bank_w64e.h

```cpp
#pragma once

#include "nmx_k_bank_w64c.h"

#define NMX_W64E_M 2048
#define NMX_W64E_TILE_FLOATS (2 * 32 * 72)
#define NMX_W64E_TWA_FLOATS (2 * 32 * 64)
#define NMX_W64E_H_FLOATS 2048

static inline int nmx_w64e_fixed(int n_spectra) { return n_spectra * NMX_W64E_H_FLOATS + NMX_W64E_TWA_FLOATS; }
static inline bool nmx_w64e_fits(int n_spectra) {
  return n_spectra >= 1 && nmx_w64_pair_waves(nmx_w64e_fixed(n_spectra), NMX_W64E_TILE_FLOATS) >= 4;
}
static inline bool nmx_w64e_notch_ok(const NmxBankArgs& b) {
  return nmx_w64_pair_shape_ok(b) && b.pad_mode != 0 && b.n_filters == 1 && b.W + 2 * b.pad_half <= NMX_W64E_M && nmx_w64e_fits(1);
}
static inline bool nmx_w64e_notch_w1000(const NmxBankArgs& b) {
  return b.pad_mode != 0 && b.W == 1000 && b.pad_half == 499 && b.n_edge >= 499;
}

#if !defined(NMX_HOST_EMU) && defined(NMX_LDS_ASM)

template <int DIR, int MM>
NMX_DEV nmx_c2 nmx_mul_w32(nmx_c2 a) {
  constexpr float C[22] = {1.f, 0.98078528040323043f, 0.92387953251128674f, 0.83146961230254524f, 0.70710678118654752f,
                           0.55557023301960218f, 0.38268343236508977f, 0.19509032201612825f, 0.f, -0.19509032201612825f,
                           -0.38268343236508977f, -0.55557023301960218f, -0.70710678118654752f, -0.83146961230254524f,
                           -0.92387953251128674f, -0.98078528040323043f, -1.f, -0.98078528040323043f, -0.92387953251128674f,
                           -0.83146961230254524f, -0.70710678118654752f, -0.55557023301960218f};
  constexpr float S[22] = {0.f, 0.19509032201612825f, 0.38268343236508977f, 0.55557023301960218f, 0.70710678118654752f,
                           0.83146961230254524f, 0.92387953251128674f, 0.98078528040323043f, 1.f, 0.98078528040323043f,
                           0.92387953251128674f, 0.83146961230254524f, 0.70710678118654752f, 0.55557023301960218f,
                           0.38268343236508977f, 0.19509032201612825f, 0.f, -0.19509032201612825f, -0.38268343236508977f,
                           -0.55557023301960218f, -0.70710678118654752f, -0.83146961230254524f};
  if constexpr (MM == 0) return a;
  else if constexpr (MM == 8) return nmx_mul_i<DIR>(a);
  else if constexpr (MM == 16) return -a;
  else if constexpr (MM == 4) return nmx_pk_mul_k(nmx_add_ib<DIR>(a, a), NMX_K_H8);
  else if constexpr (MM == 12) return nmx_pk_mul_k(nmx_add_ib<-DIR>(a, a), -NMX_K_H8);
  else if constexpr (MM == 20) return nmx_pk_mul_k(nmx_add_ib<DIR>(a, a), -NMX_K_H8);
  else return nmx_cmul_k<(DIR < 0)>(a, C[MM], S[MM]);
}

template <int JA, int FULL>
NMX_DEV void nmx_dft32_fwd_col(nmx_c2* v) {
  nmx_c2 a0 = v[JA], a1 = v[JA + 8], a2, a3;
  if (FULL) {
    a2 = v[JA + 16]; a3 = v[JA + 24];
    nmx_dft4<-1>(a0, a1, a2, a3);
  } else {
    const nmx_c2 s = a0 + a1, d = a0 - a1;
    a2 = d;
    a3 = nmx_add_ib<+1>(a0, a1);
    a1 = nmx_add_ib<-1>(a0, a1);
    a0 = s;
  }
  v[JA] = a0;
  v[JA + 8] = nmx_mul_w32<-1, JA>(a1);
  v[JA + 16] = nmx_mul_w32<-1, 2 * JA>(a2);
  v[JA + 24] = nmx_mul_w32<-1, 3 * JA>(a3);
}
template <int FULL>
NMX_DEV void nmx_dft32_fwd(nmx_c2* v) {
  nmx_dft32_fwd_col<0, FULL>(v); nmx_dft32_fwd_col<1, FULL>(v); nmx_dft32_fwd_col<2, FULL>(v); nmx_dft32_fwd_col<3, FULL>(v);
  nmx_dft32_fwd_col<4, FULL>(v); nmx_dft32_fwd_col<5, FULL>(v); nmx_dft32_fwd_col<6, FULL>(v); nmx_dft32_fwd_col<7, FULL>(v);
  nmx_dft8<-1>(v);
  nmx_dft8<-1>(v + 8);
  nmx_dft8<-1>(v + 16);
  nmx_dft8<-1>(v + 24);
}
template <int JA>
NMX_DEV void nmx_dft32_inv_col(nmx_c2* v) {
  const nmx_c2 a0 = v[JA], a1 = nmx_mul_w32<+1, JA>(v[JA + 8]), a2 = nmx_mul_w32<+1, 2 * JA>(v[JA + 16]),
               a3 = nmx_mul_w32<+1, 3 * JA>(v[JA + 24]);
  const nmx_c2 s02 = a0 + a2, d02 = a0 - a2, s13 = a1 + a3, d13 = a1 - a3;
  v[JA] = s02 + s13;
  v[JA + 8] = nmx_add_ib<+1>(d02, d13);
}
NMX_DEV void nmx_dft32_inv(nmx_c2* v) {
  nmx_dft8<+1>(v);
  nmx_dft8<+1>(v + 8);
  nmx_dft8<+1>(v + 16);
  nmx_dft8<+1>(v + 24);
  nmx_dft32_inv_col<0>(v); nmx_dft32_inv_col<1>(v); nmx_dft32_inv_col<2>(v); nmx_dft32_inv_col<3>(v);
  nmx_dft32_inv_col<4>(v); nmx_dft32_inv_col<5>(v); nmx_dft32_inv_col<6>(v); nmx_dft32_inv_col<7>(v);
}

constexpr int nmx_w64e_p1(int i) { return 8 * 72 * (4 * (i & 7) + (i >> 3)); }
template <int... I> NMX_DEV void nmx_w64e_rd1(nmx_c2* v, unsigned a, std::integer_sequence<int, I...>) { ((v[I] = nmx_ds_read_b64<nmx_w64e_p1(I)>(a)), ...); }
template <int... I> NMX_DEV void nmx_w64e_wr1(const nmx_c2* v, unsigned a, std::integer_sequence<int, I...>) { (nmx_ds_write_b64<nmx_w64e_p1(I)>(a, v[I]), ...); }
template <int I0, int... I> NMX_DEV void nmx_w64e_rdt16(nmx_c2* v, unsigned a, std::integer_sequence<int, I...>) { ((v[I] = nmx_ds_read_b64<512 * (I0 + I)>(a)), ...); }
#define NMX_W64E_SEQ32 std::make_integer_sequence<int, 32>{}
#define NMX_W64E_SEQ16 std::make_integer_sequence<int, 16>{}

template <int FULL>
NMX_DEV void nmx_w64e_forward(nmx_c2* v, const NmxW64cLane& Ln) {
  nmx_dft32_fwd<FULL>(v);
  {
    nmx_c2 w[16];
    nmx_w64e_rdt16<0>(w, Ln.twa, NMX_W64E_SEQ16);
    NMX_SCHED_FENCE();
    NMX_UNROLL
    for (int i = 1; i < 16; ++i) v[i] = nmx_cmul_tw<0>(v[i], w[i]);
    nmx_w64e_rdt16<16>(w, Ln.twa, NMX_W64E_SEQ16);
    NMX_SCHED_FENCE();
    NMX_UNROLL
    for (int i = 0; i < 16; ++i) v[16 + i] = nmx_cmul_tw<0>(v[16 + i], w[i]);
  }
  nmx_w64e_wr1(v, Ln.a1, NMX_W64E_SEQ32);
  NMX_SCHED_FENCE();
  nmx_w64c_rd2(v, Ln.a2, NMX_W64E_SEQ32);
  NMX_SCHED_FENCE();
  NMX_UNROLL
  for (int g = 0; g < 4; ++g) {
    nmx_dft8<-1>(v + 8 * g);
    NMX_UNROLL
    for (int q = 1; q < 8; ++q) v[8 * g + q] = nmx_cmul_tw<0>(v[8 * g + q], Ln.twb[q]);
  }
  nmx_w64c_wr3(v, Ln.a2, NMX_W64E_SEQ32);
  NMX_SCHED_FENCE();
  nmx_w64c_rd4(v, Ln.a4, NMX_W64E_SEQ32);
  NMX_SCHED_FENCE();
  NMX_UNROLL
  for (int g = 0; g < 4; ++g) nmx_dft8<-1>(v + 8 * g);
}
NMX_DEV void nmx_w64e_inverse(nmx_c2* v, const NmxW64cLane& Ln) {
  NMX_UNROLL
  for (int g = 0; g < 4; ++g) {
    nmx_dft8<+1>(v + 8 * g);
    NMX_UNROLL
    for (int q = 1; q < 8; ++q) v[8 * g + q] = nmx_cmul_tw<1>(v[8 * g + q], Ln.twb[q]);
  }
  nmx_w64c_wr4(v, Ln.a4, NMX_W64E_SEQ32);
  NMX_SCHED_FENCE();
  nmx_w64c_rd3(v, Ln.a2, NMX_W64E_SEQ32);
  NMX_SCHED_FENCE();
  NMX_UNROLL
  for (int g = 0; g < 4; ++g) nmx_dft8<+1>(v + 8 * g);
  nmx_w64c_wr2(v, Ln.a2, NMX_W64E_SEQ32);
  NMX_SCHED_FENCE();
  nmx_w64e_rd1(v, Ln.a1, NMX_W64E_SEQ32);
  {
    nmx_c2 w[16];
    nmx_w64e_rdt16<0>(w, Ln.twa, NMX_W64E_SEQ16);
    NMX_SCHED_FENCE();
    NMX_UNROLL
    for (int i = 1; i < 16; ++i) v[i] = nmx_cmul_tw<1>(v[i], w[i]);
    nmx_w64e_rdt16<16>(w, Ln.twa, NMX_W64E_SEQ16);
    NMX_SCHED_FENCE();
    NMX_UNROLL
    for (int i = 0; i < 16; ++i) v[16 + i] = nmx_cmul_tw<1>(v[16 + i], w[i]);
  }
  nmx_dft32_inv(v);
}

NMX_DEV void nmx_w64e_reflect_lane(const NmxBankArgs& A, int l, unsigned* rt) {
  const int W = A.W, h = A.pad_half, ne = A.n_edge;
  NMX_UNROLL
  for (int i = 0; i < 16; ++i) {
    unsigned word = 0;
    NMX_UNROLL
    for (int u = 0; u < 2; ++u) {
      const int m = l + 64 * (2 * i + u);
      const int j = m < W + h ? m : (m >= NMX_W64E_M - h ? m - NMX_W64E_M : (1 << 20));
      unsigned e = 0xfffcu;
      if (j < 0) { if (-j <= ne) e = (unsigned)(4 * -j) | 1u; }
      else if (j < W) e = (unsigned)(4 * j);
      else if (j < W + h) { const int rr = j - (W - 1); if (rr <= ne) e = (unsigned)(4 * (W - 1 - rr)) | 2u; }
      word |= e << (16 * u);
    }
    rt[i] = word;
  }
}

template <int J, int WC, int HC, bool CLEAN>
NMX_DEV nmx_c2 nmx_w64e_reflect_reg(const nmx_rsrc r1, const nmx_rsrc r2, int l, nmx_c2 x0_2, nmx_c2 xl_2) {
  constexpr int m0 = 64 * J, M = NMX_W64E_M;
  auto ld = [&](int off) -> nmx_c2 {
    nmx_c2 x = nmx_mk2(__uint_as_float(__builtin_amdgcn_raw_buffer_load_b32(r1, off, 0, 0)),
                       __uint_as_float(__builtin_amdgcn_raw_buffer_load_b32(r2, off, 0, 0)));
    if (CLEAN) x = nmx_mk2(nmx_clean_bl(x.x), nmx_clean_bl(x.y));
    return x;
  };
  nmx_c2 acc = nmx_mk2(0.f, 0.f);
  if constexpr (m0 < WC) acc = ld(4 * l + 4 * m0);
  if constexpr (m0 + 63 >= WC && m0 < WC + HC) {
    static_assert(2 * (WC - 1) - m0 - 63 >= 0, "reflection beyond the window");
    const nmx_c2 t = xl_2 - ld(4 * (63 - l) + 4 * (2 * (WC - 1) - m0 - 63));
    if constexpr (m0 >= WC && m0 + 63 < WC + HC) acc = t;
    else acc = (l >= WC - m0 && l < WC + HC - m0) ? t : acc;
  }
  if constexpr (m0 + 63 >= M - HC) {
    const nmx_c2 t = x0_2 - ld(4 * (63 - l) + 4 * (M - m0 - 63));
    if constexpr (m0 >= M - HC) acc = t;
    else acc = (l >= M - HC - m0) ? t : acc;
  }
  return acc;
}
template <int WC, int HC, bool CLEAN, int... J>
NMX_DEV void nmx_w64e_reflect_fixed(nmx_c2* v, const nmx_rsrc r1, const nmx_rsrc r2, int l, nmx_c2 x0_2, nmx_c2 xl_2,
                                    std::integer_sequence<int, J...>) {
  ((v[J] = nmx_w64e_reflect_reg<J, WC, HC, CLEAN>(r1, r2, l, x0_2, xl_2)), ...);
}

template <int NJ>
NMX_DEV nmx_c2 nmx_w64e_pair_scale(nmx_c2* v) {
  float m1 = 0.f, m2 = 0.f;
  NMX_UNROLL
  for (int j = 0; j < NJ; ++j) { m1 = fmaxf(m1, fabsf(v[j].x)); m2 = fmaxf(m2, fabsf(v[j].y)); }
  m1 = nmx_wave_reduce(m1, 0.f, [](float a_, float b_) { return fmaxf(a_, b_); });
  m2 = nmx_wave_reduce(m2, 0.f, [](float a_, float b_) { return fmaxf(a_, b_); });
  int e = 0;
  if (m1 > 0.f && m2 > 0.f) {
    e = __builtin_amdgcn_frexp_expf(m1) - __builtin_amdgcn_frexp_expf(m2);
    e = e < -60 ? -60 : (e > 60 ? 60 : e);
  }
  NMX_UNROLL
  for (int j = 0; j < NJ; ++j) v[j].y = __builtin_amdgcn_ldexpf(v[j].y, e);
  return nmx_mk2(m1 > 0.f ? 1.f : 0.f, m2 > 0.f ? __builtin_amdgcn_ldexpf(1.f, -e) : 0.f);
}

struct NmxW64eNotchHalf {
  const float* x;
  long long ch_stride, win_stride;
  const long long* starts;
  float* y_out;
  const float* hg;
  int clean_on_load, residual;
};
struct NmxW64eFusedArgs {
  NmxBankW64Args f;
  NmxW64eNotchHalf n;
};

template <int PAD, int WC = 0, int HC = 0, int FUSE = 0>
NMX_DEV void nmx_bank_w64e_item(const NmxBankW64Args& AA, int w, int c, const NmxW64cLane& Ln, const float* htab,
                                const unsigned* rt, const NmxW64eNotchHalf* N = nullptr) {
  static_assert(!FUSE || (PAD && WC), "the fused item is the notch of a compile-time shape");
  w = nmx_uniform_i(w);
  c = nmx_uniform_i(c);
  const NmxBankArgs& A = AA.b;
  const int W = A.W;
  const int l = (int)(threadIdx.x & 63);
  const bool two = c + 1 < A.n_channels;
  float* out_row = A.out ? A.out + (long long)w * A.n_outputs : nullptr;
  const float* x = A.x;
  long long ch_stride = A.ch_stride, win_stride = A.win_stride;
  const long long* starts = A.starts;
  int clean_on_load = A.clean_on_load, residual = A.residual;
  float* y_out = A.y_out;
  if constexpr (FUSE != 0) {
    x = N->x; ch_stride = N->ch_stride; win_stride = N->win_stride; starts = N->starts;
    clean_on_load = N->clean_on_load; residual = N->residual; y_out = N->y_out;
  }
  const float* src = x + (long long)c * ch_stride + (long long)w * win_stride + (starts ? nmx_uniform_ll(starts[w]) : 0ll);
  nmx_c2 v[32];
  const nmx_rsrc r1 = nmx_make_rsrc(src, 4 * W);
  const nmx_rsrc r2 = nmx_make_rsrc(src + ch_stride, two ? 4 * W : 0);
  constexpr int NJ = PAD ? 32 : 16;

  if (PAD && WC) {
    nmx_c2 x0 = nmx_mk2(__uint_as_float(__builtin_amdgcn_raw_buffer_load_b32(r1, 0, 0, 0)),
                        __uint_as_float(__builtin_amdgcn_raw_buffer_load_b32(r2, 0, 0, 0)));
    nmx_c2 xl = nmx_mk2(__uint_as_float(__builtin_amdgcn_raw_buffer_load_b32(r1, 4 * (WC - 1), 0, 0)),
                        __uint_as_float(__builtin_amdgcn_raw_buffer_load_b32(r2, 4 * (WC - 1), 0, 0)));
    if (clean_on_load) {
      x0 = nmx_mk2(nmx_clean_bl(x0.x), nmx_clean_bl(x0.y));
      xl = nmx_mk2(nmx_clean_bl(xl.x), nmx_clean_bl(xl.y));
      nmx_w64e_reflect_fixed<WC, HC, true>(v, r1, r2, l, x0 + x0, xl + xl, NMX_W64E_SEQ32);
    } else {
      nmx_w64e_reflect_fixed<WC, HC, false>(v, r1, r2, l, x0 + x0, xl + xl, NMX_W64E_SEQ32);
    }
  } else if (PAD) {
    NMX_UNROLL
    for (int j = 0; j < 32; ++j) {
      const unsigned e = (rt[j >> 1] >> (16 * (j & 1))) & 0xffffu;
      const int off = (int)(e & 0xfffcu);
      v[j].x = __uint_as_float(__builtin_amdgcn_raw_buffer_load_b32(r1, off, 0, 0));
      v[j].y = __uint_as_float(__builtin_amdgcn_raw_buffer_load_b32(r2, off, 0, 0));
    }
    nmx_c2 x0 = nmx_mk2(__uint_as_float(__builtin_amdgcn_raw_buffer_load_b32(r1, 0, 0, 0)),
                        __uint_as_float(__builtin_amdgcn_raw_buffer_load_b32(r2, 0, 0, 0)));
    nmx_c2 xl = nmx_mk2(__uint_as_float(__builtin_amdgcn_raw_buffer_load_b32(r1, 4 * (W - 1), 0, 0)),
                        __uint_as_float(__builtin_amdgcn_raw_buffer_load_b32(r2, 4 * (W - 1), 0, 0)));
    if (A.clean_on_load) {
      x0 = nmx_mk2(nmx_clean_bl(x0.x), nmx_clean_bl(x0.y));
      xl = nmx_mk2(nmx_clean_bl(xl.x), nmx_clean_bl(xl.y));
      NMX_UNROLL
      for (int j = 0; j < 32; ++j) v[j] = nmx_mk2(nmx_clean_bl(v[j].x), nmx_clean_bl(v[j].y));
    }
    const nmx_c2 x0_2 = x0 + x0, xl_2 = xl + xl, zero = nmx_mk2(0.f, 0.f);
    NMX_UNROLL
    for (int j = 0; j < 32; ++j) {
      const unsigned f = (rt[j >> 1] >> (16 * (j & 1))) & 3u;
      const nmx_c2 base = f == 1u ? x0_2 : (f == 2u ? xl_2 : zero);
      const float sg = f ? -1.f : 1.f;
      v[j] = nmx_c2_fma(v[j], nmx_mk2(sg, sg), base);
    }
  } else {
    NMX_UNROLL
    for (int j = 0; j < 16; ++j) {
      v[j].x = __uint_as_float(__builtin_amdgcn_raw_buffer_load_b32(r1, 4 * l + 256 * j, 0, 0));
      v[j].y = __uint_as_float(__builtin_amdgcn_raw_buffer_load_b32(r2, 4 * l + 256 * j, 0, 0));
    }
    if (A.clean_on_load) {
      NMX_UNROLL
      for (int j = 0; j < 16; ++j) v[j] = nmx_mk2(nmx_clean_bl(v[j].x), nmx_clean_bl(v[j].y));
    }
    if (A.dcf) {
      const nmx_c2 dd = nmx_mk2(A.dcf[c], two ? A.dcf[c + 1] : 0.f);
      NMX_UNROLL
      for (int j = 0; j < 16; ++j) {
        if (64 * j + 63 < W) v[j] += dd;
        else if (l + 64 * j < W) v[j] += dd;
      }
    }
  }
  constexpr bool KEEP = PAD && WC;
  nmx_c2 keep[KEEP ? 16 : 1];
  if constexpr (KEEP) {
    NMX_UNROLL
    for (int j = 0; j < 16; ++j) keep[j] = v[j];
  }
  nmx_c2 unscale = nmx_w64e_pair_scale<NJ>(v);

  nmx_c2 hg[FUSE == 1 ? 16 : 1];
  if constexpr (FUSE == 1) {
    const nmx_rsrc rg = nmx_make_rsrc(N->hg, 4 * NMX_W64E_H_FLOATS);
    NMX_UNROLL
    for (int i = 0; i < 16; ++i) hg[i] = __builtin_bit_cast(nmx_c2, __builtin_amdgcn_raw_buffer_load_b64(rg, 8 * l + 512 * i, 0, 0));
  }
  nmx_w64e_forward<PAD>(v, Ln);
  const unsigned h_addr = nmx_lds_addr(htab) + 8u * (unsigned)l;

  if (PAD) {
    {
      nmx_c2 h[16];
      if constexpr (FUSE == 1) {
        NMX_UNROLL
        for (int i = 0; i < 16; ++i) h[i] = hg[i];
      } else {
        nmx_w64e_rdt16<0>(h, h_addr + (FUSE ? (unsigned)A.n_filters * (NMX_W64E_H_FLOATS * 4u) : 0u), NMX_W64E_SEQ16);
        NMX_SCHED_FENCE();
      }
      NMX_UNROLL
      for (int i = 0; i < 16; ++i) {
        v[2 * i] = nmx_pk_mul_lo(v[2 * i], h[i]);
        v[2 * i + 1] = nmx_pk_mul_hi(v[2 * i + 1], h[i]);
      }
    }
    nmx_w64e_inverse(v, Ln);
    float* d = y_out + ((long long)w * A.n_channels + c) * W;
    const nmx_rsrc s1 = nmx_make_rsrc(d, 4 * W);
    const nmx_rsrc s2 = nmx_make_rsrc(d + W, two ? 4 * W : 0);
    NMX_UNROLL
    for (int j = 0; j < 16; ++j) {
      nmx_c2 y = v[j] * unscale;
      if (residual) {
        if constexpr (KEEP) {
          y = keep[j] - y;
        } else {
          nmx_c2 xw = nmx_mk2(__uint_as_float(__builtin_amdgcn_raw_buffer_load_b32(r1, 4 * l + 256 * j, 0, 0)),
                              __uint_as_float(__builtin_amdgcn_raw_buffer_load_b32(r2, 4 * l + 256 * j, 0, 0)));
          if (A.clean_on_load) xw = nmx_mk2(nmx_clean_bl(xw.x), nmx_clean_bl(xw.y));
          y = xw - y;
        }
      }
      __builtin_amdgcn_raw_buffer_store_b32(__float_as_uint(y.x), s1, 4 * l + 256 * j, 0, 0);
      __builtin_amdgcn_raw_buffer_store_b32(__float_as_uint(y.y), s2, 4 * l + 256 * j, 0, 0);
      if constexpr (FUSE != 0) v[j] = y;
    }
    if constexpr (FUSE == 0) {
      return;
    } else {
      NMX_UNROLL
      for (int j = 0; j < 16; ++j) {
        if (!two) v[j].y = 0.f;
        if (64 * j + 63 >= WC && l + 64 * j >= WC) v[j] = nmx_mk2(0.f, 0.f);
      }
      if (A.dcf) {
        const nmx_c2 dd = nmx_mk2(A.dcf[c], two ? A.dcf[c + 1] : 0.f);
        NMX_UNROLL
        for (int j = 0; j < 16; ++j) {
          if (64 * j + 63 < WC) v[j] += dd;
          else if (l + 64 * j < WC) v[j] += dd;
        }
      }
      unscale = nmx_w64e_pair_scale<16>(v);
      nmx_w64e_forward<0>(v, Ln);
    }
  }

  nmx_c2 z[32];
  NMX_UNROLL
  for (int i = 0; i < 32; ++i) z[i] = v[i];
  const int nf = A.n_filters;
  for (int fi = 0; fi < nf; ++fi) {
    const NmxFilterDev& F = A.f[fi];
    {
      nmx_c2 h[16];
      nmx_w64e_rdt16<0>(h, h_addr + (unsigned)fi * (NMX_W64E_H_FLOATS * 4u), NMX_W64E_SEQ16);
      NMX_SCHED_FENCE();
      NMX_UNROLL
      for (int i = 0; i < 16; ++i) {
        v[2 * i] = nmx_pk_mul_lo(z[2 * i], h[i]);
        v[2 * i + 1] = nmx_pk_mul_hi(z[2 * i + 1], h[i]);
      }
    }
    nmx_w64e_inverse(v, Ln);
    NMX_UNROLL
    for (int j = 0; j < 16; ++j) v[j] = v[j] * unscale;
    nmx_w64c_epilogue(AA, F, v, w, c, l, two, out_row);
  }
}
#endif
```

### py_neuromodulation_amd/csrc/nmx_w64.hip

```cpp
#include <hip/hip_runtime.h>

#include <cstdlib>

#include "nmx_k_bank_w64.h"
#include "nmx_k_bank_w64p.h"
#include "nmx_k_bank_w64x2.h"
#include "nmx_k_bank_w64c.h"
#include "nmx_k_bank_w64d.h"
#include "nmx_k_bank_w64e.h"

#if !defined(NMX_LDS_ASM)
#error "compile with -DNMX_LDS_ASM=1"
#endif

extern __shared__ __attribute__((aligned(16))) float nmx_smem_w64[];

static void nmx_w64_allow_lds();

struct NmxW64PairGeom {
  int nw, grid, chunk, n_windows, n_pairs;
  size_t lds;
};
static NmxW64PairGeom nmx_w64_pair_geom(int fixed, int tile, int cap, int n_items, int C, int n_cu) {
  NmxW64PairGeom g;
  g.n_windows = n_items / C;
  g.n_pairs = g.n_windows * ((C + 1) / 2);
  g.nw = nmx_w64_pair_waves(fixed, tile);
  if (g.nw > cap) g.nw = cap;
  if (g.n_pairs < 2048) g.nw = 2;
  g.lds = (size_t)(fixed + g.nw * tile) * 4;
  g.grid = n_cu > 0 ? n_cu : 256;
  if (g.grid * g.nw > g.n_pairs) g.grid = (g.n_pairs + g.nw - 1) / g.nw;
  g.chunk = (g.n_pairs + g.grid * g.nw - 1) / (g.grid * g.nw);
  return g;
}

__global__ void __launch_bounds__(64, 3) nmx_kern_bank_w64_rd64(const NmxBankW64Args A) {
  const int item = blockIdx.x;
  nmx_bank_w64_item<0, 0, 1>(A, item / A.b.n_channels, item % A.b.n_channels, nmx_smem_w64, nullptr);
}
__global__ void __launch_bounds__(64, 2) nmx_kern_notch_w64_rd64(const NmxBankW64Args A) {
  const int item = blockIdx.x;
  nmx_bank_w64_item<1, 0, 0>(A, item / A.b.n_channels, item % A.b.n_channels, nmx_smem_w64, nullptr);
}

template <int HALF>
__global__ void __launch_bounds__(64 * 8) nmx_kern_bank_w64pp_rd64(const NmxBankW64Args A0, int n_items, int x_floats) {
  typedef const NmxBankW64Args __attribute__((address_space(4)))* nmx_karg_p;
  nmx_karg_p Ap = (nmx_karg_p)__builtin_amdgcn_kernarg_segment_ptr();
  float* tab = nmx_smem_w64;
  const int n = NMX_W64_N, tab_floats = ((const NmxBankW64Args*)Ap)->b.n_filters * 2 * n;
  {
    const NmxBankW64Args& A = *(const NmxBankW64Args*)Ap;
    for (int i = threadIdx.x; i < tab_floats; i += blockDim.x) {
      const int fi = i / (2 * n), j = i - fi * 2 * n;
      tab[i] = (j & 1) ? A.Hd[fi][j >> 1] : A.Hs[fi][j >> 1];
    }
    for (int i = threadIdx.x; i < NMX_W64_TWL_FLOATS; i += blockDim.x) tab[tab_floats + i] = A.twl[i];
  }
  __syncthreads();
  const int wave = __builtin_amdgcn_readfirstlane((int)(threadIdx.x >> 6)), nw = blockDim.x >> 6;
  float* mine = nmx_smem_w64 + tab_floats + NMX_W64_TWL_FLOATS + wave * x_floats;
#pragma nounroll
  for (int item = blockIdx.x * nw + wave; item < n_items; item += gridDim.x * nw) {
    asm volatile("" : "+s"(Ap));
    const NmxBankW64Args& A = *(const NmxBankW64Args*)Ap;
    nmx_bank_w64_item_pipe<HALF>(A, item / A.b.n_channels, item % A.b.n_channels, mine, tab);
  }
}

__global__ void __launch_bounds__(256, 3) nmx_kern_notch_w64q_rd64(const NmxBankW64Args A, int n_items, int x_floats) {
  float* tab = nmx_smem_w64;
  const int n = NMX_W64_N, tab_floats = 2 * n;
  for (int i = threadIdx.x; i < tab_floats; i += 256) tab[i] = i < n ? A.Hs[0][i] : A.Hd[0][i - n];
  for (int i = threadIdx.x; i < NMX_W64_TWL_FLOATS; i += 256) tab[tab_floats + i] = A.twl[i];
  __syncthreads();
  const int wave = __builtin_amdgcn_readfirstlane((int)(threadIdx.x >> 6));
  const int item = blockIdx.x * 4 + wave;
  if (item >= n_items) return;
  nmx_bank_w64_item<1, 1, 0>(A, item / A.b.n_channels, item % A.b.n_channels,
                             nmx_smem_w64 + tab_floats + NMX_W64_TWL_FLOATS + wave * x_floats, tab);
}

#ifndef NMX_NOTCH_QP_WAVES
#define NMX_NOTCH_QP_WAVES 12
#endif
__global__ void __launch_bounds__(64 * NMX_NOTCH_QP_WAVES, 3) nmx_kern_notch_w64qp_rd64(const NmxBankW64Args A0, int n_items,
                                                            int x_floats) {
  typedef const NmxBankW64Args __attribute__((address_space(4)))* nmx_karg_p;
  nmx_karg_p Ap = (nmx_karg_p)__builtin_amdgcn_kernarg_segment_ptr();
  float* tab = nmx_smem_w64;
  const int n = NMX_W64_N, tab_floats = 2 * n;
  {
    const NmxBankW64Args& A = *(const NmxBankW64Args*)Ap;
    for (int i = threadIdx.x; i < tab_floats; i += 64 * NMX_NOTCH_QP_WAVES) tab[i] = i < n ? A.Hs[0][i] : A.Hd[0][i - n];
    for (int i = threadIdx.x; i < NMX_W64_TWL_FLOATS; i += 64 * NMX_NOTCH_QP_WAVES) tab[tab_floats + i] = A.twl[i];
  }
  unsigned* rtab = (unsigned*)(nmx_smem_w64 + tab_floats + NMX_W64_TWL_FLOATS);
  nmx_w64_reflect_table(((const NmxBankW64Args*)Ap)->b, rtab, (int)threadIdx.x, 64 * NMX_NOTCH_QP_WAVES);
  __syncthreads();
  const int wave = __builtin_amdgcn_readfirstlane((int)(threadIdx.x >> 6));
  float* mine = nmx_smem_w64 + tab_floats + NMX_W64_TWL_FLOATS + 1024 + wave * x_floats;
#pragma nounroll
  for (int item = blockIdx.x * NMX_NOTCH_QP_WAVES + wave; item < n_items; item += (int)gridDim.x * NMX_NOTCH_QP_WAVES) {
    asm volatile("" : "+s"(Ap));
    const NmxBankW64Args& A = *(const NmxBankW64Args*)Ap;
    nmx_bank_w64_item<1, 1, 0>(A, item / A.b.n_channels, item % A.b.n_channels, mine, tab, rtab);
    NMX_WAVE_FENCE();
  }
}

template <int HALF>
__global__ void __launch_bounds__(64 * 8) nmx_kern_bank_w64x2_rd64(const NmxBankW64Args A0, int n_items, int x_floats, int n_tab) {
  typedef const NmxBankW64Args __attribute__((address_space(4)))* nmx_karg_p;
  nmx_karg_p Ap = (nmx_karg_p)__builtin_amdgcn_kernarg_segment_ptr();
  float* tab = nmx_smem_w64;
  const int tab_floats = n_tab * 4096;
  {
    const NmxBankW64Args& A = *(const NmxBankW64Args*)Ap;
    for (int i = threadIdx.x; i < tab_floats; i += blockDim.x) tab[i] = A.Hs[i >> 12][i & 4095];
    for (int i = threadIdx.x; i < NMX_W64_TWL_FLOATS; i += blockDim.x) tab[tab_floats + i] = A.twl[i];
    for (int i = threadIdx.x; i < 2048; i += blockDim.x) tab[tab_floats + NMX_W64_TWL_FLOATS + i] = A.tw2[i];
  }
  __syncthreads();
  const int wave = __builtin_amdgcn_readfirstlane((int)(threadIdx.x >> 6)), nw = blockDim.x >> 6;
  float* mine = nmx_smem_w64 + tab_floats + NMX_W64_TWL_FLOATS + 2048 + wave * x_floats;
#pragma nounroll
  for (int item = blockIdx.x * nw + wave; item < n_items; item += gridDim.x * nw) {
    asm volatile("" : "+s"(Ap));
    const NmxBankW64Args& A = *(const NmxBankW64Args*)Ap;
    nmx_bank_w64x2_item<HALF>(A, item / A.b.n_channels, item % A.b.n_channels, mine, tab, n_tab);
  }
}

extern "C" void nmx_w64x2_launch_rd64(const NmxBankW64Args* A, int n_items, int n_cu, hipStream_t s) {
  nmx_w64_allow_lds();
  const int nw = NMX_W64X2_WAVES, x_floats = A->lds_floats;
  const int n_tab = nmx_w64x2_lds_tables(x_floats) < A->b.n_filters ? nmx_w64x2_lds_tables(x_floats) : A->b.n_filters;
  const size_t lds = (size_t)(n_tab * 4096 + nmx_w64x2_fixed(x_floats)) * 4;
  int grid = n_cu > 0 ? n_cu : 256;
  if (grid * nw > n_items) grid = (n_items + nw - 1) / nw;
  if (A->b.W <= 2048) {
    hipLaunchKernelGGL((nmx_kern_bank_w64x2_rd64<1>), dim3(grid), dim3(64 * nw), lds, s, *A, n_items, x_floats, n_tab);
    nmxi_note_kernel("nmx_kern_bank_w64x2_rd64<1>");
  } else {
    hipLaunchKernelGGL((nmx_kern_bank_w64x2_rd64<0>), dim3(grid), dim3(64 * nw), lds, s, *A, n_items, x_floats, n_tab);
    nmxi_note_kernel("nmx_kern_bank_w64x2_rd64<0>");
  }
}

__global__ void __launch_bounds__(64 * 8) nmx_kern_bank_w64c_rd64(const NmxBankW64Args A, int n_windows, int n_pairs, int chunk) {
  float* tab = nmx_smem_w64;
  const int hf = A.b.n_filters * NMX_W64C_H_FLOATS;
  for (int i = threadIdx.x; i < hf; i += blockDim.x) tab[i] = A.hc[i];
  for (int i = threadIdx.x; i < NMX_W64C_TWA_FLOATS; i += blockDim.x) tab[hf + i] = A.twc[i];
  __syncthreads();
  const int wave = __builtin_amdgcn_readfirstlane((int)(threadIdx.x >> 6)), nw = blockDim.x >> 6;
  NmxW64cLane Ln;
  nmx_w64c_lane_setup(Ln, tab + hf + NMX_W64C_TWA_FLOATS + wave * NMX_W64C_TILE_FLOATS, tab + hf,
                      A.twc + NMX_W64C_TWA_FLOATS, (int)(threadIdx.x & 63));
  const int q0 = (blockIdx.x * nw + wave) * chunk;
  const int q1 = q0 + chunk < n_pairs ? q0 + chunk : n_pairs;
#pragma nounroll
  for (int q = q0; q < q1; ++q) {
    const int cp = q / n_windows;
    nmx_bank_w64c_item(A, q - cp * n_windows, 2 * cp, Ln, tab);
  }
}

template <int HALF>
__global__ void __launch_bounds__(64 * (HALF ? 12 : 8)) nmx_kern_bank_w64d_rd64(const NmxBankW64Args A, int n_windows,
                                                            int n_pairs, int chunk, int x_floats) {
  float* tab = nmx_smem_w64;
  const int hf = A.b.n_filters * NMX_W64D_H_FLOATS;
  for (int i = threadIdx.x; i < hf; i += blockDim.x) tab[i] = A.hc[i];
  for (int i = threadIdx.x; i < NMX_W64_TWL_FLOATS; i += blockDim.x) tab[hf + i] = A.twl[i];
  __syncthreads();
  const int wave = __builtin_amdgcn_readfirstlane((int)(threadIdx.x >> 6)), nw = blockDim.x >> 6;
  float* mine = tab + hf + NMX_W64_TWL_FLOATS + wave * x_floats;
  const int q0 = (blockIdx.x * nw + wave) * chunk;
  const int q1 = q0 + chunk < n_pairs ? q0 + chunk : n_pairs;
#pragma nounroll
  for (int q = q0; q < q1; ++q) {
    const int cp = q / n_windows;
    nmx_bank_w64d_item<HALF>(A, q - cp * n_windows, 2 * cp, mine, tab);
  }
}

extern "C" void nmx_w64d_launch_rd64(const NmxBankW64Args* A, int n_items, int n_cu, hipStream_t s) {
  nmx_w64_allow_lds();
  const int x_floats = A->lds_floats;
  const NmxW64PairGeom g = nmx_w64_pair_geom(nmx_w64d_fixed(A->b.n_filters), x_floats, A->b.W <= 512 ? 12 : 8, n_items, A->b.n_channels, n_cu);
  if (A->b.W <= 512) {
    hipLaunchKernelGGL((nmx_kern_bank_w64d_rd64<1>), dim3(g.grid), dim3(64 * g.nw), g.lds, s, *A, g.n_windows, g.n_pairs, g.chunk, x_floats);
    nmxi_note_kernel("nmx_kern_bank_w64d_rd64<1>");
  } else {
    hipLaunchKernelGGL((nmx_kern_bank_w64d_rd64<0>), dim3(g.grid), dim3(64 * g.nw), g.lds, s, *A, g.n_windows, g.n_pairs, g.chunk, x_floats);
    nmxi_note_kernel("nmx_kern_bank_w64d_rd64<0>");
  }
}

template <int PAD, int WC = 0, int HC = 0>
__global__ void __launch_bounds__(64 * 8) nmx_kern_bank_w64e_rd64(const NmxBankW64Args A0, int n_windows, int n_pairs, int chunk) {
  typedef const NmxBankW64Args __attribute__((address_space(4)))* nmx_karg_p;
  nmx_karg_p Ap = (nmx_karg_p)__builtin_amdgcn_kernarg_segment_ptr();
  float* tab = nmx_smem_w64;
  const int hf = ((const NmxBankW64Args*)Ap)->b.n_filters * NMX_W64E_H_FLOATS;
  NmxW64cLane Ln;
  unsigned rt[16];
  const int wave = __builtin_amdgcn_readfirstlane((int)(threadIdx.x >> 6)), nw = blockDim.x >> 6;
  {
    const NmxBankW64Args& A = *(const NmxBankW64Args*)Ap;
    for (int i = threadIdx.x; i < hf; i += blockDim.x) tab[i] = A.hc[i];
    for (int i = threadIdx.x; i < NMX_W64E_TWA_FLOATS; i += blockDim.x) tab[hf + i] = A.twc[i];
    nmx_w64c_lane_setup(Ln, tab + hf + NMX_W64E_TWA_FLOATS + wave * NMX_W64E_TILE_FLOATS, tab + hf,
                        A.twc + NMX_W64E_TWA_FLOATS, (int)(threadIdx.x & 63));
    if (PAD && !WC) nmx_w64e_reflect_lane(A.b, (int)(threadIdx.x & 63), rt);
  }
  __syncthreads();
  const int q0 = (blockIdx.x * nw + wave) * chunk;
  const int q1 = q0 + chunk < n_pairs ? q0 + chunk : n_pairs;
#pragma nounroll
  for (int q = q0; q < q1; ++q) {
    asm volatile("" : "+s"(Ap));
    const NmxBankW64Args& A = *(const NmxBankW64Args*)Ap;
    const int cp = q / n_windows;
    nmx_bank_w64e_item<PAD, WC, HC>(A, q - cp * n_windows, 2 * cp, Ln, tab, rt);
  }
}

template <int WC, int HC, int FUSE>
__global__ void __launch_bounds__(64 * 8) nmx_kern_notch_bank_w64e_rd64(const NmxW64eFusedArgs A0, int n_windows,
                                                            int n_pairs, int chunk) {
  typedef const NmxW64eFusedArgs __attribute__((address_space(4)))* nmx_karg_p;
  nmx_karg_p Ap = (nmx_karg_p)__builtin_amdgcn_kernarg_segment_ptr();
  float* tab = nmx_smem_w64;
  const int hff = ((const NmxW64eFusedArgs*)Ap)->f.b.n_filters * NMX_W64E_H_FLOATS;
  const int hf = hff + (FUSE == 2 ? NMX_W64E_H_FLOATS : 0);
  NmxW64cLane Ln;
  const int wave = __builtin_amdgcn_readfirstlane((int)(threadIdx.x >> 6)), nw = blockDim.x >> 6;
  {
    const NmxW64eFusedArgs& A = *(const NmxW64eFusedArgs*)Ap;
    for (int i = threadIdx.x; i < hff; i += blockDim.x) tab[i] = A.f.hc[i];
    if (FUSE == 2)
      for (int i = threadIdx.x; i < NMX_W64E_H_FLOATS; i += blockDim.x) tab[hff + i] = A.n.hg[i];
    for (int i = threadIdx.x; i < NMX_W64E_TWA_FLOATS; i += blockDim.x) tab[hf + i] = A.f.twc[i];
    nmx_w64c_lane_setup(Ln, tab + hf + NMX_W64E_TWA_FLOATS + wave * NMX_W64E_TILE_FLOATS, tab + hf,
                        A.f.twc + NMX_W64E_TWA_FLOATS, (int)(threadIdx.x & 63));
  }
  __syncthreads();
  const int q0 = (blockIdx.x * nw + wave) * chunk;
  const int q1 = q0 + chunk < n_pairs ? q0 + chunk : n_pairs;
#pragma nounroll
  for (int q = q0; q < q1; ++q) {
    asm volatile("" : "+s"(Ap));
    const NmxW64eFusedArgs& A = *(const NmxW64eFusedArgs*)Ap;
    const int cp = q / n_windows;
    nmx_bank_w64e_item<1, WC, HC, FUSE>(A.f, q - cp * n_windows, 2 * cp, Ln, tab, nullptr, &A.n);
  }
}

extern "C" void nmx_w64e_launch_fused_rd64(const NmxBankW64Args* F, const NmxBankW64Args* Nn, int g_lds, int n_items, int n_cu,
                                           hipStream_t s) {
  nmx_w64_allow_lds();
  NmxW64eFusedArgs A;
  A.f = *F;
  A.n.x = Nn->b.x; A.n.ch_stride = Nn->b.ch_stride; A.n.win_stride = Nn->b.win_stride; A.n.starts = Nn->b.starts;
  A.n.y_out = Nn->b.y_out; A.n.hg = Nn->hc; A.n.clean_on_load = Nn->b.clean_on_load; A.n.residual = Nn->b.residual;
  const NmxW64PairGeom g = nmx_w64_pair_geom(nmx_w64e_fixed(F->b.n_filters + (g_lds ? 1 : 0)), NMX_W64E_TILE_FLOATS, 8, n_items,
                                             F->b.n_channels, n_cu);
  if (g_lds) {
    hipLaunchKernelGGL((nmx_kern_notch_bank_w64e_rd64<1000, 499, 2>), dim3(g.grid), dim3(64 * g.nw), g.lds, s, A, g.n_windows, g.n_pairs, g.chunk);
    nmxi_note_kernel("nmx_kern_notch_bank_w64e_rd64<1000, 499, 2>");
  } else {
    hipLaunchKernelGGL((nmx_kern_notch_bank_w64e_rd64<1000, 499, 1>), dim3(g.grid), dim3(64 * g.nw), g.lds, s, A, g.n_windows, g.n_pairs, g.chunk);
    nmxi_note_kernel("nmx_kern_notch_bank_w64e_rd64<1000, 499, 1>");
  }
}

extern "C" void nmx_w64e_launch_rd64(const NmxBankW64Args* A, int n_items, int n_cu, hipStream_t s) {
  nmx_w64_allow_lds();
  const NmxW64PairGeom g = nmx_w64_pair_geom(nmx_w64e_fixed(A->b.n_filters), NMX_W64E_TILE_FLOATS, 8, n_items, A->b.n_channels, n_cu);
  if (nmx_w64e_notch_w1000(A->b)) {
    hipLaunchKernelGGL((nmx_kern_bank_w64e_rd64<1, 1000, 499>), dim3(g.grid), dim3(64 * g.nw), g.lds, s, *A, g.n_windows, g.n_pairs, g.chunk);
    nmxi_note_kernel("nmx_kern_bank_w64e_rd64<1, 1000, 499>");
  } else if (A->b.pad_mode != 0) {
    hipLaunchKernelGGL((nmx_kern_bank_w64e_rd64<1>), dim3(g.grid), dim3(64 * g.nw), g.lds, s, *A, g.n_windows, g.n_pairs, g.chunk);
    nmxi_note_kernel("nmx_kern_bank_w64e_rd64<1>");
  } else {
    hipLaunchKernelGGL((nmx_kern_bank_w64e_rd64<0>), dim3(g.grid), dim3(64 * g.nw), g.lds, s, *A, g.n_windows, g.n_pairs, g.chunk);
    nmxi_note_kernel("nmx_kern_bank_w64e_rd64<0>");
  }
}

extern "C" void nmx_w64c_launch_rd64(const NmxBankW64Args* A, int n_items, int n_cu, hipStream_t s) {
  nmx_w64_allow_lds();
  const NmxW64PairGeom g = nmx_w64_pair_geom(nmx_w64c_fixed(A->b.n_filters), NMX_W64C_TILE_FLOATS, 8, n_items, A->b.n_channels, n_cu);
  hipLaunchKernelGGL(nmx_kern_bank_w64c_rd64, dim3(g.grid), dim3(64 * g.nw), g.lds, s, *A, g.n_windows, g.n_pairs, g.chunk);
  nmxi_note_kernel("nmx_kern_bank_w64c_rd64");
}

extern "C" void nmx_w64_launch_rd64(const NmxBankW64Args* A, int n_items, size_t lds, int n_cu, hipStream_t s) {
  nmx_w64_allow_lds();
  const int x_floats = A->lds_floats;
  if (n_items >= 4096 && A->pipelined) {
    const int nw = NMX_W64P_WAVES, tab_floats = A->b.n_filters * 2 * NMX_W64_N;
    const size_t ldsp = (size_t)(tab_floats + NMX_W64_TWL_FLOATS + nw * x_floats) * 4;
    int grid = n_cu > 0 ? n_cu : 256;
    if (grid * nw > n_items) grid = (n_items + nw - 1) / nw;
    if (A->b.W <= 1024) {
      hipLaunchKernelGGL((nmx_kern_bank_w64pp_rd64<1>), dim3(grid), dim3(64 * nw), ldsp, s, *A, n_items, x_floats);
      nmxi_note_kernel("nmx_kern_bank_w64pp_rd64<1>");
    } else {
      hipLaunchKernelGGL((nmx_kern_bank_w64pp_rd64<0>), dim3(grid), dim3(64 * nw), ldsp, s, *A, n_items, x_floats);
      nmxi_note_kernel("nmx_kern_bank_w64pp_rd64<0>");
    }
  } else if (A->b.pad_mode != 0 && n_items >= 3 * 256 * 4 * 8) {
    const size_t ldsp = (size_t)(2 * NMX_W64_N + NMX_W64_TWL_FLOATS + 1024 + NMX_NOTCH_QP_WAVES * x_floats) * 4;
    hipLaunchKernelGGL(nmx_kern_notch_w64qp_rd64, dim3((12 / NMX_NOTCH_QP_WAVES) * 256), dim3(64 * NMX_NOTCH_QP_WAVES), ldsp, s, *A, n_items, x_floats);
    nmxi_note_kernel("nmx_kern_notch_w64qp_rd64");
  } else if (A->b.pad_mode != 0 && n_items >= 1024) {
    const size_t ldsq = (size_t)(2 * NMX_W64_N + NMX_W64_TWL_FLOATS + 4 * x_floats) * 4;
    hipLaunchKernelGGL(nmx_kern_notch_w64q_rd64, dim3((n_items + 3) / 4), dim3(256), ldsq, s, *A, n_items, x_floats);
    nmxi_note_kernel("nmx_kern_notch_w64q_rd64");
  } else if (A->b.pad_mode == 0) {
    hipLaunchKernelGGL(nmx_kern_bank_w64_rd64, dim3(n_items), dim3(64), lds, s, *A);
    nmxi_note_kernel("nmx_kern_bank_w64_rd64");
  } else {
    hipLaunchKernelGGL(nmx_kern_notch_w64_rd64, dim3(n_items), dim3(64), lds, s, *A);
    nmxi_note_kernel("nmx_kern_notch_w64_rd64");
  }
}

static void nmx_w64_allow_lds() {
  static unsigned long long seen = 0;
  if (!nmx_first_on_device(seen)) return;
  const void* kernels[] = {(const void*)nmx_kern_bank_w64_rd64, (const void*)nmx_kern_notch_w64_rd64,
                           (const void*)nmx_kern_bank_w64pp_rd64<0>, (const void*)nmx_kern_bank_w64pp_rd64<1>,
                           (const void*)nmx_kern_notch_w64q_rd64, (const void*)nmx_kern_notch_w64qp_rd64,
                           (const void*)nmx_kern_bank_w64x2_rd64<0>, (const void*)nmx_kern_bank_w64x2_rd64<1>,
                           (const void*)nmx_kern_bank_w64c_rd64, (const void*)nmx_kern_bank_w64d_rd64<0>,
                           (const void*)nmx_kern_bank_w64d_rd64<1>, (const void*)nmx_kern_bank_w64e_rd64<0>,
                           (const void*)nmx_kern_bank_w64e_rd64<1>, (const void*)nmx_kern_bank_w64e_rd64<1, 1000, 499>,
                           (const void*)nmx_kern_notch_bank_w64e_rd64<1000, 499, 1>, (const void*)nmx_kern_notch_bank_w64e_rd64<1000, 499, 2>};
  for (const void* k : kernels) (void)hipFuncSetAttribute(k, hipFuncAttributeMaxDynamicSharedMemorySize, 160 * 1024);
}
```

Baseline: 163,400 windows/s.

## Shrink w64c/w64e LDS transpose tiles to 8-row groups and raise waves

Rewrites the LDS transpose exchanges in the w64c and w64e FFT filter-bank kernels so each wave writes and reads one 8-row group at a time through a per-group 8x72 tile, instead of staging all 24 or 32 rows at once. Each wave's LDS tile shrinks by a factor of three or four, so the launcher can fit more waves per block: 12 for w64c and 7 for w64e, up from 8. The admission check still uses the old full-size tile so kernel selection does not change. It also adds host-side logging of the pair geometry. The per-group exchange adds extra LDS write/read round trips and a temporary register buffer, which may increase register pressure.

```diff
diff --git a/py_neuromodulation_amd/csrc/nmx_api.hip b/py_neuromodulation_amd/csrc/nmx_api.hip
--- a/py_neuromodulation_amd/csrc/nmx_api.hip
+++ b/py_neuromodulation_amd/csrc/nmx_api.hip
@@ -138,11 +138,21 @@
 
 static thread_local int g_stage = 0;
 static thread_local std::string g_stage_kernels[16];
+static thread_local const char* g_last_kernel = "";
 extern "C" void nmxi_note_kernel(const char* name) {
+  g_last_kernel = name;
   std::string& s = g_stage_kernels[g_stage & 15];
   if (s.find(name) != std::string::npos) return;
   if (!s.empty()) s += " + ";
   s += name;
+}
+#define NMX_GEOM_SLOT 15
+extern "C" void nmxi_note_pair_geom(int n_pairs, int grid, int nw) {
+  std::string& s = g_stage_kernels[NMX_GEOM_SLOT];
+  const std::string e = std::string(g_last_kernel) + ": " + std::to_string(n_pairs) + " pairs, " + std::to_string(grid) + " x " + std::to_string(nw) + " waves";
+  if (s.find(e) != std::string::npos) return;
+  if (!s.empty()) s += " + ";
+  s += e;
 }
 static void be_stage(int st) { g_stage = st; }
 static void be_stage_reset() { for (auto& s : g_stage_kernels) s.clear(); }
diff --git a/py_neuromodulation_amd/csrc/nmx_common.h b/py_neuromodulation_amd/csrc/nmx_common.h
--- a/py_neuromodulation_amd/csrc/nmx_common.h
+++ b/py_neuromodulation_amd/csrc/nmx_common.h
@@ -54,6 +54,7 @@
 #define NMX_RESTRICT __restrict__
 #define NMX_GLOBAL_FENCE() __threadfence_block()
 extern "C" void nmxi_note_kernel(const char* name);
+extern "C" void nmxi_note_pair_geom(int n_pairs, int grid, int nw);
 static inline bool nmx_first_on_device(unsigned long long& seen) {
   int d = 0;
   if (hipGetDevice(&d) != hipSuccess || d < 0 || d > 63) return true;
diff --git a/py_neuromodulation_amd/csrc/nmx_engine.inc b/py_neuromodulation_amd/csrc/nmx_engine.inc
--- a/py_neuromodulation_amd/csrc/nmx_engine.inc
+++ b/py_neuromodulation_amd/csrc/nmx_engine.inc
@@ -229,6 +229,7 @@
   int w_in = 0;
   be_timer_t timers[ST_COUNT];
   std::string kernels[ST_COUNT];
+  std::string pair_geom;
   nmx_norm* norm = nullptr;
   nmx_proj* proj = nullptr;
   bool dc_ok = false;
diff --git a/py_neuromodulation_amd/csrc/nmx_engine_run.inc b/py_neuromodulation_amd/csrc/nmx_engine_run.inc
--- a/py_neuromodulation_amd/csrc/nmx_engine_run.inc
+++ b/py_neuromodulation_amd/csrc/nmx_engine_run.inc
@@ -106,7 +106,10 @@
   if (!sharp_side && (rc = launch_sharp_stage(P, par, nw, d_out, s, tev))) return rc;
   P.sched.end_main(b);
   be_stage(ST_BATCH);
-  if (timed) for (int i = 0; i < ST_PROJ; ++i) P.kernels[i] = be_stage_kernels(i);
+  if (timed) {
+    for (int i = 0; i < ST_PROJ; ++i) P.kernels[i] = be_stage_kernels(i);
+    P.pair_geom = be_stage_kernels(15);
+  }
   return be_check_launch();
 }
 
@@ -387,6 +390,7 @@
   if ((rc = run_prep_stages(P, v, 1, s))) return rc;
   be_stage(ST_BATCH);
   for (int i = 0; i < ST_PROJ; ++i) P.kernels[i] = be_stage_kernels(i);
+  P.pair_geom = be_stage_kernels(15);
   be_d2h_async(yf.data(), v.x, yf.size() * sizeof(float), s);
   if ((rc = be_sync(s))) return rc;
   for (int c = 0; c < C; ++c)
@@ -426,6 +430,7 @@
   launch_fir_stage(P, P.bank, A, C, s, false, true);
   be_stage(ST_BATCH);
   for (int i = 0; i < ST_PROJ; ++i) P.kernels[i] = be_stage_kernels(i);
+  P.pair_geom = be_stage_kernels(15);
   be_d2h_async(yf.data(), P.sharp.swy[0].p, yf.size() * sizeof(float), s);
   if ((rc = be_sync(s))) return rc;
   for (size_t i = 0; i < yf.size(); ++i) y[i] = (double)yf[i];
@@ -557,8 +562,8 @@
 
 int nmx_last_kernels(nmx_plan* plan, int which, char* buf, int64_t n) {
   Plan* P = (Plan*)plan;
-  if (!P || !buf || n < 1 || which < ST_PREP || which >= ST_COUNT) return nmx_fail(NMX_E_INVALID, "bad argument");
-  std::string k = P->kernels[which];
+  if (!P || !buf || n < 1 || which < ST_PREP || which > ST_COUNT) return nmx_fail(NMX_E_INVALID, "bad argument");
+  std::string k = which == ST_COUNT ? P->pair_geom : P->kernels[which];
   if (which == ST_BURSTS && P->bursts.sparse_count)
     k += (k.empty() ? "" : ",") + std::string("env_tail_rows=") + std::to_string(P->bursts.env_tail_rows) + "/" + std::to_string(P->bursts.env_rows);
   const size_t m = std::min<size_t>(k.size(), (size_t)n - 1);
diff --git a/py_neuromodulation_amd/csrc/nmx_k_bank_w64c.h b/py_neuromodulation_amd/csrc/nmx_k_bank_w64c.h
--- a/py_neuromodulation_amd/csrc/nmx_k_bank_w64c.h
+++ b/py_neuromodulation_amd/csrc/nmx_k_bank_w64c.h
@@ -3,7 +3,9 @@
 #include "nmx_k_bank_w64.h"
 
 #define NMX_W64C_M 1536
-#define NMX_W64C_TILE_FLOATS (2 * 24 * 72)
+#define NMX_W64_GROUP_TILE_FLOATS (2 * 8 * 72)
+#define NMX_W64C_TILE_FLOATS NMX_W64_GROUP_TILE_FLOATS
+#define NMX_W64C_ADMIT_TILE_FLOATS (2 * 24 * 72)
 #define NMX_W64C_TWA_FLOATS (2 * 24 * 64)
 #define NMX_W64C_TWB_FLOATS (2 * 8 * 8)
 #define NMX_W64C_H_FLOATS 1536
@@ -12,7 +14,7 @@
 static inline int nmx_w64_pair_waves(int fixed, int tile) { return (NMX_W64_LDS_FLOATS - fixed) / tile; }
 static inline int nmx_w64c_fixed(int n_filters) { return n_filters * NMX_W64C_H_FLOATS + NMX_W64C_TWA_FLOATS; }
 static inline bool nmx_w64c_fits(int n_filters) {
-  return n_filters >= 1 && nmx_w64_pair_waves(nmx_w64c_fixed(n_filters), NMX_W64C_TILE_FLOATS) >= 6;
+  return n_filters >= 1 && nmx_w64_pair_waves(nmx_w64c_fixed(n_filters), NMX_W64C_ADMIT_TILE_FLOATS) >= 6;
 }
 
 #if !defined(NMX_HOST_EMU) && defined(NMX_LDS_ASM)
@@ -124,19 +126,40 @@
   nmx_dft24_inv_col<4>(v); nmx_dft24_inv_col<5>(v); nmx_dft24_inv_col<6>(v); nmx_dft24_inv_col<7>(v);
 }
 
-constexpr int nmx_w64c_p1(int i) { return 8 * 72 * (3 * (i & 7) + (i >> 3)); }
-constexpr int nmx_w64c_p2(int i) { return 8 * (576 * (i >> 3) + 8 * (i & 7)); }
-constexpr int nmx_w64c_p3(int i) { return 8 * (576 * (i >> 3) + 9 * (i & 7)); }
-constexpr int nmx_w64c_p4(int i) { return 8 * (576 * (i >> 3) + (i & 7)); }
-template <int... I> NMX_DEV void nmx_w64c_rd1(nmx_c2* v, unsigned a, std::integer_sequence<int, I...>) { ((v[I] = nmx_ds_read_b64<nmx_w64c_p1(I)>(a)), ...); }
-template <int... I> NMX_DEV void nmx_w64c_rd2(nmx_c2* v, unsigned a, std::integer_sequence<int, I...>) { ((v[I] = nmx_ds_read_b64<nmx_w64c_p2(I)>(a)), ...); }
-template <int... I> NMX_DEV void nmx_w64c_rd3(nmx_c2* v, unsigned a, std::integer_sequence<int, I...>) { ((v[I] = nmx_ds_read_b64<nmx_w64c_p3(I)>(a)), ...); }
-template <int... I> NMX_DEV void nmx_w64c_rd4(nmx_c2* v, unsigned a, std::integer_sequence<int, I...>) { ((v[I] = nmx_ds_read_b64<nmx_w64c_p4(I)>(a)), ...); }
-template <int... I> NMX_DEV void nmx_w64c_wr1(const nmx_c2* v, unsigned a, std::integer_sequence<int, I...>) { (nmx_ds_write_b64<nmx_w64c_p1(I)>(a, v[I]), ...); }
-template <int... I> NMX_DEV void nmx_w64c_wr2(const nmx_c2* v, unsigned a, std::integer_sequence<int, I...>) { (nmx_ds_write_b64<nmx_w64c_p2(I)>(a, v[I]), ...); }
-template <int... I> NMX_DEV void nmx_w64c_wr3(const nmx_c2* v, unsigned a, std::integer_sequence<int, I...>) { (nmx_ds_write_b64<nmx_w64c_p3(I)>(a, v[I]), ...); }
-template <int... I> NMX_DEV void nmx_w64c_wr4(const nmx_c2* v, unsigned a, std::integer_sequence<int, I...>) { (nmx_ds_write_b64<nmx_w64c_p4(I)>(a, v[I]), ...); }
+template <int G> constexpr int nmx_w64g_ka(int i) { return G * (i & 7) + (i >> 3); }
+template <int G> constexpr int nmx_w64g_p1(int i) { return 8 * 72 * (nmx_w64g_ka<G>(i) & 7); }
+constexpr int nmx_w64g_p2(int i) { return 8 * (8 * (i & 7)); }
+constexpr int nmx_w64g_p3(int i) { return 8 * (9 * (i & 7)); }
+constexpr int nmx_w64g_p4(int i) { return 8 * (i & 7); }
+template <int G, int GRP, int I> NMX_DEV void nmx_w64g_rd1_reg(nmx_c2* v, unsigned a) {
+  if constexpr ((nmx_w64g_ka<G>(I) >> 3) == GRP) v[I] = nmx_ds_read_b64<nmx_w64g_p1<G>(I)>(a);
+}
+template <int G, int GRP, int I> NMX_DEV void nmx_w64g_wr1_reg(const nmx_c2* v, unsigned a) {
+  if constexpr ((nmx_w64g_ka<G>(I) >> 3) == GRP) nmx_ds_write_b64<nmx_w64g_p1<G>(I)>(a, v[I]);
+}
+template <int G, int GRP, int... I> NMX_DEV void nmx_w64g_rd1(nmx_c2* v, unsigned a, std::integer_sequence<int, I...>) { (nmx_w64g_rd1_reg<G, GRP, I>(v, a), ...); }
+template <int G, int GRP, int... I> NMX_DEV void nmx_w64g_wr1(const nmx_c2* v, unsigned a, std::integer_sequence<int, I...>) { (nmx_w64g_wr1_reg<G, GRP, I>(v, a), ...); }
+template <int... I> NMX_DEV void nmx_w64g_rd2(nmx_c2* v, unsigned a, std::integer_sequence<int, I...>) { ((v[I] = nmx_ds_read_b64<nmx_w64g_p2(I)>(a)), ...); }
+template <int... I> NMX_DEV void nmx_w64g_rd3(nmx_c2* v, unsigned a, std::integer_sequence<int, I...>) { ((v[I] = nmx_ds_read_b64<nmx_w64g_p3(I)>(a)), ...); }
+template <int... I> NMX_DEV void nmx_w64g_rd4(nmx_c2* v, unsigned a, std::integer_sequence<int, I...>) { ((v[I] = nmx_ds_read_b64<nmx_w64g_p4(I)>(a)), ...); }
+template <int... I> NMX_DEV void nmx_w64g_wr2(const nmx_c2* v, unsigned a, std::integer_sequence<int, I...>) { (nmx_ds_write_b64<nmx_w64g_p2(I)>(a, v[I]), ...); }
+template <int... I> NMX_DEV void nmx_w64g_wr3(const nmx_c2* v, unsigned a, std::integer_sequence<int, I...>) { (nmx_ds_write_b64<nmx_w64g_p3(I)>(a, v[I]), ...); }
+template <int... I> NMX_DEV void nmx_w64g_wr4(const nmx_c2* v, unsigned a, std::integer_sequence<int, I...>) { (nmx_ds_write_b64<nmx_w64g_p4(I)>(a, v[I]), ...); }
+#define NMX_W64G_SEQ8 std::make_integer_sequence<int, 8>{}
+template <int G, int... GRP> NMX_DEV void nmx_w64g_xch_ab(const nmx_c2* v, nmx_c2* b, unsigned a1, unsigned a2, std::integer_sequence<int, GRP...>) {
+  ((nmx_w64g_wr1<G, GRP>(v, a1, std::make_integer_sequence<int, 8 * G>{}), nmx_w64g_rd2(b + 8 * GRP, a2, NMX_W64G_SEQ8)), ...);
+}
+template <int G, int... GRP> NMX_DEV void nmx_w64g_xch_ba(const nmx_c2* v, nmx_c2* b, unsigned a1, unsigned a2, std::integer_sequence<int, GRP...>) {
+  ((nmx_w64g_wr2(v + 8 * GRP, a2, NMX_W64G_SEQ8), nmx_w64g_rd1<G, GRP>(b, a1, std::make_integer_sequence<int, 8 * G>{})), ...);
+}
+template <int... GRP> NMX_DEV void nmx_w64g_xch_bc(nmx_c2* v, unsigned a2, unsigned a4, std::integer_sequence<int, GRP...>) {
+  ((nmx_w64g_wr3(v + 8 * GRP, a2, NMX_W64G_SEQ8), nmx_w64g_rd4(v + 8 * GRP, a4, NMX_W64G_SEQ8)), ...);
+}
+template <int... GRP> NMX_DEV void nmx_w64g_xch_cb(nmx_c2* v, unsigned a2, unsigned a4, std::integer_sequence<int, GRP...>) {
+  ((nmx_w64g_wr4(v + 8 * GRP, a4, NMX_W64G_SEQ8), nmx_w64g_rd3(v + 8 * GRP, a2, NMX_W64G_SEQ8)), ...);
+}
 template <int... I> NMX_DEV void nmx_w64c_rdt(nmx_c2* v, unsigned a, std::integer_sequence<int, I...>) { ((v[I] = nmx_ds_read_b64<512 * I>(a)), ...); }
+template <int I0, int... I> NMX_DEV void nmx_w64c_rdt8(nmx_c2* v, unsigned a, std::integer_sequence<int, I...>) { ((v[I] = nmx_ds_read_b64<512 * (I0 + I)>(a)), ...); }
 
 struct NmxW64cLane {
   unsigned a1, a2, a4;
@@ -144,6 +167,7 @@
   nmx_c2 twb[8];
 };
 #define NMX_W64C_SEQ24 std::make_integer_sequence<int, 24>{}
+#define NMX_W64C_SEQ3 std::make_integer_sequence<int, 3>{}
 
 NMX_DEV void nmx_w64c_forward(nmx_c2* v, const NmxW64cLane& Ln) {
   nmx_c2 w[24];
@@ -152,19 +176,20 @@
   nmx_dft24_fwd(v);
   NMX_UNROLL
   for (int i = 1; i < 24; ++i) v[i] = nmx_cmul_tw<0>(v[i], w[i]);
-  nmx_w64c_wr1(v, Ln.a1, NMX_W64C_SEQ24);
-  NMX_SCHED_FENCE();
-  nmx_w64c_rd2(v, Ln.a2, NMX_W64C_SEQ24);
-  NMX_SCHED_FENCE();
+  {
+    nmx_c2 b[24];
+    nmx_w64g_xch_ab<3>(v, b, Ln.a1, Ln.a2, NMX_W64C_SEQ3);
+    NMX_SCHED_FENCE();
+    NMX_UNROLL
+    for (int i = 0; i < 24; ++i) v[i] = b[i];
+  }
   NMX_UNROLL
   for (int g = 0; g < 3; ++g) {
     nmx_dft8<-1>(v + 8 * g);
     NMX_UNROLL
     for (int q = 1; q < 8; ++q) v[8 * g + q] = nmx_cmul_tw<0>(v[8 * g + q], Ln.twb[q]);
   }
-  nmx_w64c_wr3(v, Ln.a2, NMX_W64C_SEQ24);
-  NMX_SCHED_FENCE();
-  nmx_w64c_rd4(v, Ln.a4, NMX_W64C_SEQ24);
+  nmx_w64g_xch_bc(v, Ln.a2, Ln.a4, NMX_W64C_SEQ3);
   NMX_SCHED_FENCE();
   NMX_UNROLL
   for (int g = 0; g < 3; ++g) nmx_dft8<-1>(v + 8 * g);
@@ -176,20 +201,24 @@
     NMX_UNROLL
     for (int q = 1; q < 8; ++q) v[8 * g + q] = nmx_cmul_tw<1>(v[8 * g + q], Ln.twb[q]);
   }
-  nmx_w64c_wr4(v, Ln.a4, NMX_W64C_SEQ24);
+  nmx_w64g_xch_cb(v, Ln.a2, Ln.a4, NMX_W64C_SEQ3);
   NMX_SCHED_FENCE();
-  nmx_w64c_rd3(v, Ln.a2, NMX_W64C_SEQ24);
-  NMX_SCHED_FENCE();
   NMX_UNROLL
   for (int g = 0; g < 3; ++g) nmx_dft8<+1>(v + 8 * g);
-  nmx_w64c_wr2(v, Ln.a2, NMX_W64C_SEQ24);
-  NMX_SCHED_FENCE();
-  nmx_c2 w[24];
-  nmx_w64c_rd1(v, Ln.a1, NMX_W64C_SEQ24);
-  nmx_w64c_rdt(w, Ln.twa, NMX_W64C_SEQ24);
-  NMX_SCHED_FENCE();
-  NMX_UNROLL
-  for (int i = 1; i < 24; ++i) v[i] = nmx_cmul_tw<1>(v[i], w[i]);
+  {
+    nmx_c2 b[24];
+    nmx_w64g_xch_ba<3>(v, b, Ln.a1, Ln.a2, NMX_W64C_SEQ3);
+    NMX_UNROLL
+    for (int k = 0; k < 3; ++k) {
+      nmx_c2 w[8];
+      if (k == 0) nmx_w64c_rdt8<0>(w, Ln.twa, NMX_W64G_SEQ8);
+      if (k == 1) nmx_w64c_rdt8<8>(w, Ln.twa, NMX_W64G_SEQ8);
+      if (k == 2) nmx_w64c_rdt8<16>(w, Ln.twa, NMX_W64G_SEQ8);
+      NMX_SCHED_FENCE();
+      NMX_UNROLL
+      for (int i = 0; i < 8; ++i) v[8 * k + i] = (8 * k + i) ? nmx_cmul_tw<1>(b[8 * k + i], w[i]) : b[0];
+    }
+  }
   nmx_dft24_inv(v);
 }
 
diff --git a/py_neuromodulation_amd/csrc/nmx_k_bank_w64e.h b/py_neuromodulation_amd/csrc/nmx_k_bank_w64e.h
--- a/py_neuromodulation_amd/csrc/nmx_k_bank_w64e.h
+++ b/py_neuromodulation_amd/csrc/nmx_k_bank_w64e.h
@@ -3,13 +3,14 @@
 #include "nmx_k_bank_w64c.h"
 
 #define NMX_W64E_M 2048
-#define NMX_W64E_TILE_FLOATS (2 * 32 * 72)
+#define NMX_W64E_TILE_FLOATS NMX_W64_GROUP_TILE_FLOATS
+#define NMX_W64E_ADMIT_TILE_FLOATS (2 * 32 * 72)
 #define NMX_W64E_TWA_FLOATS (2 * 32 * 64)
 #define NMX_W64E_H_FLOATS 2048
 
 static inline int nmx_w64e_fixed(int n_spectra) { return n_spectra * NMX_W64E_H_FLOATS + NMX_W64E_TWA_FLOATS; }
 static inline bool nmx_w64e_fits(int n_spectra) {
-  return n_spectra >= 1 && nmx_w64_pair_waves(nmx_w64e_fixed(n_spectra), NMX_W64E_TILE_FLOATS) >= 4;
+  return n_spectra >= 1 && nmx_w64_pair_waves(nmx_w64e_fixed(n_spectra), NMX_W64E_ADMIT_TILE_FLOATS) >= 4;
 }
 static inline bool nmx_w64e_notch_ok(const NmxBankArgs& b) {
   return nmx_w64_pair_shape_ok(b) && b.pad_mode != 0 && b.n_filters == 1 && b.W + 2 * b.pad_half <= NMX_W64E_M && nmx_w64e_fits(1);
@@ -85,12 +86,11 @@
   nmx_dft32_inv_col<4>(v); nmx_dft32_inv_col<5>(v); nmx_dft32_inv_col<6>(v); nmx_dft32_inv_col<7>(v);
 }
 
-constexpr int nmx_w64e_p1(int i) { return 8 * 72 * (4 * (i & 7) + (i >> 3)); }
-template <int... I> NMX_DEV void nmx_w64e_rd1(nmx_c2* v, unsigned a, std::integer_sequence<int, I...>) { ((v[I] = nmx_ds_read_b64<nmx_w64e_p1(I)>(a)), ...); }
-template <int... I> NMX_DEV void nmx_w64e_wr1(const nmx_c2* v, unsigned a, std::integer_sequence<int, I...>) { (nmx_ds_write_b64<nmx_w64e_p1(I)>(a, v[I]), ...); }
+
 template <int I0, int... I> NMX_DEV void nmx_w64e_rdt16(nmx_c2* v, unsigned a, std::integer_sequence<int, I...>) { ((v[I] = nmx_ds_read_b64<512 * (I0 + I)>(a)), ...); }
 #define NMX_W64E_SEQ32 std::make_integer_sequence<int, 32>{}
 #define NMX_W64E_SEQ16 std::make_integer_sequence<int, 16>{}
+#define NMX_W64E_SEQ4 std::make_integer_sequence<int, 4>{}
 
 template <int FULL>
 NMX_DEV void nmx_w64e_forward(nmx_c2* v, const NmxW64cLane& Ln) {
@@ -106,19 +106,20 @@
     NMX_UNROLL
     for (int i = 0; i < 16; ++i) v[16 + i] = nmx_cmul_tw<0>(v[16 + i], w[i]);
   }
-  nmx_w64e_wr1(v, Ln.a1, NMX_W64E_SEQ32);
-  NMX_SCHED_FENCE();
-  nmx_w64c_rd2(v, Ln.a2, NMX_W64E_SEQ32);
-  NMX_SCHED_FENCE();
+  {
+    nmx_c2 b[32];
+    nmx_w64g_xch_ab<4>(v, b, Ln.a1, Ln.a2, NMX_W64E_SEQ4);
+    NMX_SCHED_FENCE();
+    NMX_UNROLL
+    for (int i = 0; i < 32; ++i) v[i] = b[i];
+  }
   NMX_UNROLL
   for (int g = 0; g < 4; ++g) {
     nmx_dft8<-1>(v + 8 * g);
     NMX_UNROLL
     for (int q = 1; q < 8; ++q) v[8 * g + q] = nmx_cmul_tw<0>(v[8 * g + q], Ln.twb[q]);
   }
-  nmx_w64c_wr3(v, Ln.a2, NMX_W64E_SEQ32);
-  NMX_SCHED_FENCE();
-  nmx_w64c_rd4(v, Ln.a4, NMX_W64E_SEQ32);
+  nmx_w64g_xch_bc(v, Ln.a2, Ln.a4, NMX_W64E_SEQ4);
   NMX_SCHED_FENCE();
   NMX_UNROLL
   for (int g = 0; g < 4; ++g) nmx_dft8<-1>(v + 8 * g);
@@ -130,15 +131,16 @@
     NMX_UNROLL
     for (int q = 1; q < 8; ++q) v[8 * g + q] = nmx_cmul_tw<1>(v[8 * g + q], Ln.twb[q]);
   }
-  nmx_w64c_wr4(v, Ln.a4, NMX_W64E_SEQ32);
+  nmx_w64g_xch_cb(v, Ln.a2, Ln.a4, NMX_W64E_SEQ4);
   NMX_SCHED_FENCE();
-  nmx_w64c_rd3(v, Ln.a2, NMX_W64E_SEQ32);
-  NMX_SCHED_FENCE();
   NMX_UNROLL
   for (int g = 0; g < 4; ++g) nmx_dft8<+1>(v + 8 * g);
-  nmx_w64c_wr2(v, Ln.a2, NMX_W64E_SEQ32);
-  NMX_SCHED_FENCE();
-  nmx_w64e_rd1(v, Ln.a1, NMX_W64E_SEQ32);
+  {
+    nmx_c2 b[32];
+    nmx_w64g_xch_ba<4>(v, b, Ln.a1, Ln.a2, NMX_W64E_SEQ4);
+    NMX_UNROLL
+    for (int i = 0; i < 32; ++i) v[i] = b[i];
+  }
   {
     nmx_c2 w[16];
     nmx_w64e_rdt16<0>(w, Ln.twa, NMX_W64E_SEQ16);
diff --git a/py_neuromodulation_amd/csrc/nmx_w64.hip b/py_neuromodulation_amd/csrc/nmx_w64.hip
--- a/py_neuromodulation_amd/csrc/nmx_w64.hip
+++ b/py_neuromodulation_amd/csrc/nmx_w64.hip
@@ -34,6 +34,7 @@
   g.chunk = (g.n_pairs + g.grid * g.nw - 1) / (g.grid * g.nw);
   return g;
 }
+static void nmx_w64_note_geom(const NmxW64PairGeom& g) { nmxi_note_pair_geom(g.n_pairs, g.grid, g.nw); }
 
 __global__ void __launch_bounds__(64, 3) nmx_kern_bank_w64_rd64(const NmxBankW64Args A) {
   const int item = blockIdx.x;
@@ -149,7 +150,7 @@
   }
 }
 
-__global__ void __launch_bounds__(64 * 8) nmx_kern_bank_w64c_rd64(const NmxBankW64Args A, int n_windows, int n_pairs, int chunk) {
+__global__ void __launch_bounds__(64 * 12) nmx_kern_bank_w64c_rd64(const NmxBankW64Args A, int n_windows, int n_pairs, int chunk) {
   float* tab = nmx_smem_w64;
   const int hf = A.b.n_filters * NMX_W64C_H_FLOATS;
   for (int i = threadIdx.x; i < hf; i += blockDim.x) tab[i] = A.hc[i];
@@ -194,12 +195,15 @@
   if (A->b.W <= 512) {
     hipLaunchKernelGGL((nmx_kern_bank_w64d_rd64<1>), dim3(g.grid), dim3(64 * g.nw), g.lds, s, *A, g.n_windows, g.n_pairs, g.chunk, x_floats);
     nmxi_note_kernel("nmx_kern_bank_w64d_rd64<1>");
+    nmx_w64_note_geom(g);
   } else {
     hipLaunchKernelGGL((nmx_kern_bank_w64d_rd64<0>), dim3(g.grid), dim3(64 * g.nw), g.lds, s, *A, g.n_windows, g.n_pairs, g.chunk, x_floats);
     nmxi_note_kernel("nmx_kern_bank_w64d_rd64<0>");
-  }
-}
-
+    nmx_w64_note_geom(g);
+  }
+}
+
+#define NMX_W64E_WAVES 7
 template <int PAD, int WC = 0, int HC = 0>
 __global__ void __launch_bounds__(64 * 8) nmx_kern_bank_w64e_rd64(const NmxBankW64Args A0, int n_windows, int n_pairs, int chunk) {
   typedef const NmxBankW64Args __attribute__((address_space(4)))* nmx_karg_p;
@@ -267,37 +271,43 @@
   A.f = *F;
   A.n.x = Nn->b.x; A.n.ch_stride = Nn->b.ch_stride; A.n.win_stride = Nn->b.win_stride; A.n.starts = Nn->b.starts;
   A.n.y_out = Nn->b.y_out; A.n.hg = Nn->hc; A.n.clean_on_load = Nn->b.clean_on_load; A.n.residual = Nn->b.residual;
-  const NmxW64PairGeom g = nmx_w64_pair_geom(nmx_w64e_fixed(F->b.n_filters + (g_lds ? 1 : 0)), NMX_W64E_TILE_FLOATS, 8, n_items,
+  const NmxW64PairGeom g = nmx_w64_pair_geom(nmx_w64e_fixed(F->b.n_filters + (g_lds ? 1 : 0)), NMX_W64E_TILE_FLOATS, NMX_W64E_WAVES, n_items,
                                              F->b.n_channels, n_cu);
   if (g_lds) {
     hipLaunchKernelGGL((nmx_kern_notch_bank_w64e_rd64<1000, 499, 2>), dim3(g.grid), dim3(64 * g.nw), g.lds, s, A, g.n_windows, g.n_pairs, g.chunk);
     nmxi_note_kernel("nmx_kern_notch_bank_w64e_rd64<1000, 499, 2>");
+    nmx_w64_note_geom(g);
   } else {
     hipLaunchKernelGGL((nmx_kern_notch_bank_w64e_rd64<1000, 499, 1>), dim3(g.grid), dim3(64 * g.nw), g.lds, s, A, g.n_windows, g.n_pairs, g.chunk);
     nmxi_note_kernel("nmx_kern_notch_bank_w64e_rd64<1000, 499, 1>");
+    nmx_w64_note_geom(g);
   }
 }
 
 extern "C" void nmx_w64e_launch_rd64(const NmxBankW64Args* A, int n_items, int n_cu, hipStream_t s) {
   nmx_w64_allow_lds();
-  const NmxW64PairGeom g = nmx_w64_pair_geom(nmx_w64e_fixed(A->b.n_filters), NMX_W64E_TILE_FLOATS, 8, n_items, A->b.n_channels, n_cu);
+  const NmxW64PairGeom g = nmx_w64_pair_geom(nmx_w64e_fixed(A->b.n_filters), NMX_W64E_TILE_FLOATS, NMX_W64E_WAVES, n_items, A->b.n_channels, n_cu);
   if (nmx_w64e_notch_w1000(A->b)) {
     hipLaunchKernelGGL((nmx_kern_bank_w64e_rd64<1, 1000, 499>), dim3(g.grid), dim3(64 * g.nw), g.lds, s, *A, g.n_windows, g.n_pairs, g.chunk);
     nmxi_note_kernel("nmx_kern_bank_w64e_rd64<1, 1000, 499>");
+    nmx_w64_note_geom(g);
   } else if (A->b.pad_mode != 0) {
     hipLaunchKernelGGL((nmx_kern_bank_w64e_rd64<1>), dim3(g.grid), dim3(64 * g.nw), g.lds, s, *A, g.n_windows, g.n_pairs, g.chunk);
     nmxi_note_kernel("nmx_kern_bank_w64e_rd64<1>");
+    nmx_w64_note_geom(g);
   } else {
     hipLaunchKernelGGL((nmx_kern_bank_w64e_rd64<0>), dim3(g.grid), dim3(64 * g.nw), g.lds, s, *A, g.n_windows, g.n_pairs, g.chunk);
     nmxi_note_kernel("nmx_kern_bank_w64e_rd64<0>");
+    nmx_w64_note_geom(g);
   }
 }
 
 extern "C" void nmx_w64c_launch_rd64(const NmxBankW64Args* A, int n_items, int n_cu, hipStream_t s) {
   nmx_w64_allow_lds();
-  const NmxW64PairGeom g = nmx_w64_pair_geom(nmx_w64c_fixed(A->b.n_filters), NMX_W64C_TILE_FLOATS, 8, n_items, A->b.n_channels, n_cu);
+  const NmxW64PairGeom g = nmx_w64_pair_geom(nmx_w64c_fixed(A->b.n_filters), NMX_W64C_TILE_FLOATS, 12, n_items, A->b.n_channels, n_cu);
   hipLaunchKernelGGL(nmx_kern_bank_w64c_rd64, dim3(g.grid), dim3(64 * g.nw), g.lds, s, *A, g.n_windows, g.n_pairs, g.chunk);
   nmxi_note_kernel("nmx_kern_bank_w64c_rd64");
+  nmx_w64_note_geom(g);
 }
 
 extern "C" void nmx_w64_launch_rd64(const NmxBankW64Args* A, int n_items, size_t lds, int n_cu, hipStream_t s) {
```

Measured after the change: 165,600 windows/s (median of 6 runs). +1.3%, better.
